# TACJu/Axial-VS

Hardware: AMD Instinct MI355X
Metric: axial-trajectory-attn fwd frames/sec at [B=1,T=4,C=256,H=W=64]; 1/2/4/8 GPU (higher is better)
Workload: dtype f16

## Files before the change

axial_vs_amd/_lib.py:

```python
from __future__ import annotations

import ctypes as C
import os
import threading
from typing import Optional

_HERE = os.path.dirname(os.path.abspath(__file__))
LIB_PATH = os.environ.get("AXVS_LIB_PATH") or os.path.join(_HERE, "libaxvs.so")

AXVS_F16 = 0
AXVS_BF16 = 1
AXVS_F32 = 2
AXVS_U8 = 3
DTYPES = {"f16": AXVS_F16, "fp16": AXVS_F16, "float16": AXVS_F16, "bf16": AXVS_BF16, "bfloat16": AXVS_BF16}

_fp = C.c_void_p


class AxvsTrajParams(C.Structure):
    _fields_ = [(n, _fp) for n in ("q_w", "q_b", "k_w", "k_b", "v_w", "v_b", "proj_q_w", "proj_q_b",
                                   "proj_kv_w", "proj_kv_b", "proj_w", "proj_b")]


class AxvsAxialLayerParams(C.Structure):
# ... 136 lines not shown
class AxvsCnxDownParams(C.Structure):
    _fields_ = [(n, _fp) for n in CNX_DOWN_FIELDS]


class AxvsCnxBlockParams(C.Structure):
    _fields_ = [(n, _fp) for n in CNX_BLOCK_FIELDS]


class AxvsCnxCfg(C.Structure):
    _fields_ = [(n, C.c_int) for n in ("N", "H", "W")] + [(n, C.c_int * 4) for n in ("dims", "depths", "h", "w")] + [("v2", C.c_int)]


class AxvsMsdaParams(C.Structure):
    _fields_ = [(n, _fp) for n in ("value_proj_w", "value_proj_b", "sampling_offsets_w", "sampling_offsets_b",
                                   "attention_weights_w", "attention_weights_b", "output_proj_w", "output_proj_b")]


class AxvsMsdaLayerParams(C.Structure):
    _fields_ = [("self_attn", AxvsMsdaParams)] + [(n, _fp) for n in ("norm1_w", "norm1_b", "linear1_w", "linear1_b", "linear2_w",
                                                                      "linear2_b", "norm2_w", "norm2_b")]


class AxvsConvGnParams(C.Structure):
    _fields_ = [(n, _fp) for n in ("conv_w", "conv_b", "gn_w", "gn_b")]


class AxvsFfnParams(C.Structure):
    _fields_ = [(n, _fp) for n in ("norm1_w", "norm1_b", "linear1_w", "linear1_b", "linear2_w", "linear2_b", "norm2_w", "norm2_b")]


class AxvsFpnLevelParams(C.Structure):
    _fields_ = [(n, _fp) for n in ("lateral_w", "lateral_gn_w", "lateral_gn_b", "output_w", "output_gn_w", "output_gn_b", "mask_w", "mask_b")]


def ptrs(ts) -> C.Array:
    return (C.c_void_p * len(ts))(*[None if t is None else t.data_ptr() for t in ts])


def fill(cls, ptrs):
    ptrs = list(ptrs)
    s, n = _fill(cls, ptrs, 0)
    if n != len(ptrs):
        raise ValueError(f"{cls.__name__} takes {n} pointers, got {len(ptrs)}")
    return s


def _fill(cls, ptrs, i):
    s = cls()
    for name, t in cls._fields_:
        if issubclass(t, C.Structure):
            v, i = _fill(t, ptrs, i)
        elif issubclass(t, C.Array):
            v, i = t(*ptrs[i:i + t._length_]), i + t._length_
        else:
            v, i = (ptrs[i] if i < len(ptrs) else None), i + 1
        setattr(s, name, v)
    return s, i


class AxvsTestGemm(C.Structure):
    _fields_ = [("op", C.c_int), ("a", _fp), ("b", _fp), ("c", _fp), ("M", C.c_longlong), ("N", C.c_int), ("K", C.c_int),
                ("lda", C.c_longlong), ("ldb", C.c_longlong), ("ldc", C.c_longlong), ("al_a", C.c_int), ("al_b", C.c_int), ("al_c", C.c_int),
                ("a2", _fp), ("aff", _fp), ("aff_rows", C.c_int), ("ksteps", C.c_int), ("zsplits", C.c_int), ("bias", _fp), ("mul", C.c_float),
                ("relu", C.c_int), ("drop_seed", C.c_uint), ("drop_site", C.c_uint), ("drop_thr", C.c_uint), ("drop_scale", C.c_float),
                ("beta", C.c_float), ("res", _fp), ("res2", _fp), ("out16", _fp), ("kind16", C.c_int), ("zero_rows", _fp), ("db", _fp),
                ("exact", C.c_int), ("stat_part", _fp), ("stat_shift", _fp), ("stat_nblk", C.c_int), ("stat_blk0", C.c_int),
                ("stat_rows", C.c_int), ("grp_rows", C.c_int), ("grp_ld", C.c_longlong), ("variant", C.c_int)]


TEST_GEMM_OPS = {"nt": 0, "fwd": 1, "wgrad": 2, "dgrad": 3, "tn_direct": 4}


SIGNATURES = {
    "axvs_version": (C.c_int, []),
    "axvs_has_bf16": (C.c_int, []),
    "axvs_last_error": (C.c_char_p, []),
    "axvs_set_status_buffer": (C.c_int, [_fp]),
    "axvs_check_status": (C.c_int, []),
    "axvs_set_sync_buffer": (C.c_int, [_fp, C.c_size_t]),
    "axvs_profile_stages": (C.c_int, [C.POINTER(C.c_void_p), C.c_int]),
    "axvs_profile_stage_count": (C.c_int, []),
    "axvs_profile_stage_name": (C.c_char_p, [C.c_int]),
    "axvs_set_option": (C.c_int, [C.c_char_p, C.c_int]),
    "axvs_traj_packed_bytes": (C.c_size_t, [C.c_int, C.c_int]),
    "axvs_traj_pack": (C.c_int, [C.POINTER(AxvsTrajParams), _fp, C.c_int, C.c_int, C.c_int, _fp]),
    "axvs_axial_layer_packed_bytes": (C.c_size_t, [C.c_int, C.c_int, C.c_int]),
    "axvs_axial_layer_pack": (C.c_int, [C.POINTER(AxvsAxialLayerParams), _fp, C.c_int, C.c_int, C.c_int, C.c_int, _fp]),
    "axvs_traj_attn_workspace_bytes": (C.c_size_t, [C.c_int] * 5),
    "axvs_traj_attn_fwd": (C.c_int, [_fp, _fp, _fp, _fp, _fp, _fp] + [C.c_int] * 6 + [_fp, C.c_size_t, _fp]),
    "axvs_axial_layer_workspace_bytes": (C.c_size_t, [C.c_int] * 7),
    "axvs_axial_layer_fwd": (C.c_int, [_fp, _fp, _fp, _fp] + [C.c_int] * 8 + [_fp, C.c_size_t, _fp, _fp, _fp]),
    "axvs_traj_layer_packed_bytes": (C.c_size_t, [C.c_int] * 3),
    "axvs_traj_layer_pack": (C.c_int, [C.POINTER(AxvsTrajLayerParams), _fp, C.c_int, C.c_int, C.c_int, C.c_int, _fp]),
    "axvs_traj_layer_workspace_bytes": (C.c_size_t, [C.c_int] * 6),
    "axvs_traj_layer_fwd": (C.c_int, [_fp, _fp, _fp, _fp] + [C.c_int] * 7 + [_fp, C.c_size_t, _fp]),
    "axvs_axial_layer_train_saved_bytes": (C.c_size_t, [C.c_int] * 7),
    "axvs_axial_layer_train_scratch_bytes": (C.c_size_t, [C.c_int] * 8),
    "axvs_axial_layer_train_fwd": (C.c_int, [_fp, _fp, _fp, C.POINTER(AxvsAxialLayerParams)] + [C.c_int] * 7 +
                                   [C.c_float, C.c_float, C.c_uint, _fp, C.c_size_t, _fp, C.c_size_t, _fp]),
    "axvs_axial_layer_train_bwd": (C.c_int, [_fp, _fp, _fp, C.POINTER(AxvsAxialLayerParams), C.POINTER(AxvsAxialLayerParams), _fp, _fp] +
                                   [C.c_int] * 7 + [C.c_float, C.c_float, C.c_uint, C.c_int, _fp, C.c_size_t, _fp, C.c_size_t, _fp]),
    "axvs_traj_layer_train_saved_bytes": (C.c_size_t, [C.c_int] * 6),
    "axvs_traj_layer_train_scratch_bytes": (C.c_size_t, [C.c_int] * 7),
    "axvs_traj_layer_train_fwd": (C.c_int, [_fp, _fp, _fp, C.POINTER(AxvsTrajLayerParams)] + [C.c_int] * 6 +
                                  [C.c_float, C.c_float, C.c_uint, _fp, C.c_size_t, _fp, C.c_size_t, _fp]),
    "axvs_traj_layer_train_bwd": (C.c_int, [_fp, _fp, _fp, C.POINTER(AxvsTrajLayerParams), C.POINTER(AxvsTrajLayerParams), _fp, _fp] +
                                  [C.c_int] * 6 + [C.c_float, C.c_float, C.c_uint, C.c_int, _fp, C.c_size_t, _fp, C.c_size_t, _fp]),
    "axvs_cc_module_train_saved_bytes": (C.c_size_t, [C.POINTER(AxvsCCTrainCfg)]),
    "axvs_cc_module_train_scratch_bytes": (C.c_size_t, [C.POINTER(AxvsCCTrainCfg), C.c_int]),
    "axvs_cc_module_train_bn_stats_floats": (C.c_size_t, [C.POINTER(AxvsCCTrainCfg)]),
    "axvs_cc_module_train_fwd": (C.c_int, [_fp] * 5 + [C.POINTER(AxvsCCLayerParams), C.POINTER(AxvsCCHeadParams), C.POINTER(AxvsCCTrainCfg),
                                           _fp, C.c_size_t, _fp, C.c_size_t, _fp]),
    "axvs_cc_module_train_bwd": (C.c_int, [_fp] * 4 + [C.POINTER(AxvsCCLayerParams), C.POINTER(AxvsCCHeadParams), C.POINTER(AxvsCCLayerParams),
                                           C.POINTER(AxvsCCHeadGrads), _fp, C.POINTER(AxvsCCTrainCfg), _fp, C.c_size_t, _fp, C.c_size_t, _fp]),
    "axvs_cc_layers_train_fwd": (C.c_int, [_fp, _fp, C.POINTER(AxvsCCLayerParams), C.POINTER(AxvsCCTrainCfg), _fp, C.c_size_t, _fp, C.c_size_t, _fp]),
    "axvs_cc_layers_train_bwd": (C.c_int, [_fp, _fp, C.POINTER(AxvsCCLayerParams), C.POINTER(AxvsCCLayerParams), _fp, C.POINTER(AxvsCCTrainCfg),
                                           _fp, C.c_size_t, _fp, C.c_size_t, _fp]),
    "axvs_axial_pass_fwd": (C.c_int, [_fp, _fp, _fp, _fp] + [C.c_int] * 9 + [_fp, C.c_size_t, _fp]),
    "axvs_axial_layer_workspace_bytes_ex": (C.c_size_t, [C.c_int] * 9),
    "axvs_axial_layer_sine3d_workspace_bytes": (C.c_size_t, [C.c_int] * 7),
    "axvs_axial_layer_fwd_sine3d": (C.c_int, [_fp, C.POINTER(AxvsSinePos3D), _fp, _fp] + [C.c_int] * 8 + [_fp, C.c_size_t, _fp, _fp, _fp]),
    "axvs_axial_layer_strided_ok": (C.c_int, [C.c_int] * 3),
    "axvs_axial_layer_workspace_bytes_strided": (C.c_size_t, [C.c_int] * 7 + [C.c_longlong]),
    "axvs_axial_layer_fwd_sine3d_strided": (C.c_int, [_fp, C.POINTER(AxvsSinePos3D), _fp, _fp] + [C.c_int] * 8 + [C.c_longlong, _fp, C.c_size_t, _fp]),
    "axvs_ffn_workspace_bytes": (C.c_size_t, [C.c_longlong, C.c_int, C.c_int]),
    "axvs_ffn_fwd": (C.c_int, [_fp, _fp, _fp, C.c_longlong, C.c_int, C.c_int, C.c_int, C.c_int, _fp, C.c_size_t, _fp]),
    "axvs_cc_layer_packed_bytes": (C.c_size_t, []),
    "axvs_cc_layer_pack": (C.c_int, [C.POINTER(AxvsCCLayerParams), _fp, C.c_int, _fp]),
    "axvs_cc_layer_workspace_bytes": (C.c_size_t, [C.c_int] * 3),
    "axvs_cc_layer_fwd": (C.c_int, [_fp, _fp, _fp, C.c_int, C.c_int, C.c_int, C.POINTER(C.c_int), C.c_int, _fp, C.c_size_t, _fp]),
    "axvs_cc_heads_packed_bytes": (C.c_size_t, [C.c_int]),
    "axvs_cc_heads_pack": (C.c_int, [C.POINTER(AxvsCCHeadParams), _fp, C.c_int, C.c_int, _fp]),
    "axvs_cc_heads_workspace_bytes": (C.c_size_t, [C.c_int] * 3),
    "axvs_cc_heads_fwd": (C.c_int, [_fp, _fp, _fp, _fp, _fp] + [C.c_int] * 8 + [_fp, C.c_size_t, _fp]),
    "axvs_ffn_packed_bytes": (C.c_size_t, [C.c_int, C.c_int]),
    "axvs_ffn_pack": (C.c_int, [C.POINTER(AxvsFfnParams), _fp, C.c_int, C.c_int, C.c_int, _fp]),
    "axvs_ffn_packed_fwd": (C.c_int, [_fp, _fp, _fp, C.c_longlong, C.c_int, C.c_int, C.c_int, _fp, C.c_size_t, _fp]),
    "axvs_fpn_level_packed_bytes": (C.c_size_t, [C.c_int] * 3),
    "axvs_fpn_level_pack": (C.c_int, [C.POINTER(AxvsFpnLevelParams), _fp, C.c_int, C.c_int, C.c_int, C.c_int, _fp]),
    "axvs_fpn_level_workspace_bytes": (C.c_size_t, [C.c_int] * 6),
    "axvs_fpn_level_fwd": (C.c_int, [_fp, _fp, C.c_longlong, C.c_longlong, C.c_int, C.c_int, _fp, _fp, _fp] + [C.c_int] * 7 +
                           [C.c_float, C.c_int, _fp, C.c_size_t, _fp]),
    "axvs_conv1x1_gn_packed_bytes": (C.c_size_t, [C.c_int, C.c_int]),
    "axvs_conv1x1_gn_pack": (C.c_int, [C.POINTER(AxvsConvGnParams), _fp, C.c_int, C.c_int, C.c_int, _fp]),
    "axvs_conv1x1_gn_workspace_bytes": (C.c_size_t, [C.c_int] * 4),
    "axvs_conv1x1_gn_fwd": (C.c_int, [_fp, C.c_int, C.c_longlong, C.c_longlong, _fp, C.c_int, C.c_longlong, C.c_longlong, _fp] +
                            [C.c_int] * 5 + [C.c_float, C.c_int, _fp, C.c_size_t, _fp]),
    "axvs_conv1x1_gn_train_saved_bytes": (C.c_size_t, [C.c_int] * 6 + [C.c_longlong, C.c_longlong]),
    "axvs_conv1x1_gn_train_scratch_bytes": (C.c_size_t, [C.c_int] * 6),
    "axvs_conv1x1_gn_train_fwd": (C.c_int, [_fp, C.c_int, C.c_longlong, C.c_longlong, _fp, C.c_int, C.c_longlong, C.c_longlong, C.POINTER(AxvsConvGnParams)] +
                                  [C.c_int] * 5 + [C.c_float, _fp, C.c_size_t, _fp, C.c_size_t, _fp]),
    "axvs_conv1x1_gn_train_bwd": (C.c_int, [_fp, C.c_int, C.c_longlong, C.c_longlong, _fp, C.c_int, C.c_longlong, C.c_longlong, C.POINTER(AxvsConvGnParams),
                                            C.POINTER(AxvsConvGnParams), _fp] + [C.c_int] * 5 + [_fp, C.c_size_t, _fp, C.c_size_t, _fp]),
    "axvs_linear_sum_assignment": (C.c_int, [_fp, _fp, C.c_int, C.c_int, _fp]),
    "axvs_match_embds_workspace_bytes": (C.c_size_t, [C.c_int, C.c_int]),
    "axvs_match_embds": (C.c_int, [_fp, _fp, _fp, C.c_int, C.c_int, _fp, C.c_size_t, _fp]),
    "axvs_match_clips_workspace_bytes": (C.c_size_t, [C.c_int] * 4),
    "axvs_match_clips": (C.c_int, [_fp, _fp] + [C.c_int] * 4 + [_fp, C.c_size_t, _fp]),
    "axvs_linear_sum_assignment_rect": (C.c_int, [_fp, C.c_longlong, C.c_int, C.c_int, C.POINTER(C.c_int), _fp, _fp, C.c_int, _fp]),
    "axvs_video_matcher_workspace_bytes": (C.c_size_t, [C.c_int] * 4 + [C.c_longlong]),
    "axvs_video_matcher": (C.c_int, [C.POINTER(_fp), C.c_int, C.POINTER(_fp), _fp, C.c_int, _fp, C.POINTER(C.c_int)] + [C.c_int] * 4 +
                           [C.c_longlong, C.c_int, C.c_int] + [_fp] * 5 + [_fp, C.c_size_t, _fp]),
    "axvs_set_criterion_saved_bytes": (C.c_size_t, [C.c_int] * 3),
    "axvs_set_criterion_workspace_bytes": (C.c_size_t, [C.c_int] * 4 + [C.c_longlong]),
    "axvs_set_criterion_fwd": (C.c_int, [C.POINTER(_fp), C.POINTER(_fp), _fp, C.c_int, _fp, C.POINTER(C.c_int)] + [_fp] * 4 + [C.c_int] * 5 +
                               [C.c_longlong, C.c_int, C.c_int, _fp, _fp, _fp, C.c_longlong, _fp]),
# ... 181 lines not shown
```

axial_vs_amd/csrc/axvs_api.hip:

```cpp
#include <hip/hip_runtime.h>

#include <algorithm>
#include <cmath>
#include <cstdio>
#include <cstring>
#include <type_traits>

#include "axvs_infer.h"
#include "axvs_attn.h"
#include "axvs_fused.h"
#include "axvs_ffn_split.h"
#include "axvs_ffn_wide.h"
#include "axvs_misc.h"

namespace axvs {
namespace {

constexpr int kMergeSmall = 128;
thread_local int g_generic_only = 0;
thread_local int* g_status = nullptr;
thread_local volatile int* g_status_host = nullptr;
thread_local unsigned g_sync_spin_limit = axvs::kSyncSpinLimit;
thread_local long long g_row_span = 0;
thread_local int g_ffn_wide = 0;
thread_local int g_no_small_tiles = 0;
thread_local int g_ffn_split_pairs = 1;
thread_local int g_spatial_only = 0;
thread_local int g_no_ffn_fusion = 0;
thread_local int g_no_reassoc = 0;
thread_local int g_ffn_gelu = 0;
thread_local unsigned* g_sync = nullptr;
thread_local size_t g_sync_words = 0;
thread_local int g_merge_qkv_any = 0;
thread_local int g_merge_small = kMergeSmall;
thread_local int g_out_dtype = 0;
thread_local int g_no_merge_qkv = 0;
thread_local int g_no_attn_fusion = 0;

constexpr int kSmallBelow = 65;
constexpr int kMergeMid = 1;
constexpr int kQkvSplitUpto = 64;
int cu_count() {
  static thread_local int dev_seen = -1, cus = 0;
  int dev = 0;
  if (hipGetDevice(&dev) != hipSuccess) return 0;
  if (dev != dev_seen) {
    hipDeviceProp_t pr;
    if (hipGetDeviceProperties(&pr, dev) != hipSuccess) return 0;
    cus = pr.multiProcessorCount;
    dev_seen = dev;
  }
  return cus;
}

int status_gate() {
  if (g_status_host != nullptr && (*g_status_host & AXVS_STATUS_SYNC_TIMEOUT))
    return fail(AXVS_ERR_STATE, "an earlier merged q/k/v + trajectory launch gave up waiting for its sibling row tiles (status bit 2, "
                                "AXVS_STATUS_SYNC_TIMEOUT): its outputs are invalid and its sync words are not zero.  Synchronise, zero the sync words "
                                "(axvs_set_sync_buffer contract), clear the status word, then call again -- or run two launches per pass "
                                "(axvs_set_sync_buffer(NULL, 0) / option no_merge_qkv)");
  return AXVS_OK;
}

template <bool BF>
void pack_w(const float* W, u16* out, PackDim nd, PackDim kd, hipStream_t st, int n_off = 0, int n_total = 0) {
  long long total = (long long)nd.padded * kd.padded;
  hipLaunchKernelGGL((pack_weight_kernel<BF>), dim3((unsigned)((total + 255) / 256)), dim3(256), 0, st, W, out, nd, kd, n_off,
                     n_total ? n_total : nd.padded);
}
template <bool BF>
void pack_w3(const float* W, u16* out, PackDim nd, PackDim kd, hipStream_t st, int n_off = 0, int n_total = 0) {
  long long total = (long long)nd.padded * kd.padded;
  hipLaunchKernelGGL((pack_weight_split3_kernel<BF>), dim3((unsigned)((total + 255) / 256)), dim3(256), 0, st, W, out, nd, kd, n_off,
                     n_total ? n_total : nd.padded);
}

template <bool BF>
void pack_ffn(const float* n1w, const float* n1b, const float* l1w, const float* l1b, const float* l2w, const float* l2b,
              const float* n2w, const float* n2b, const LayerPacked& l, int C, int F, hipStream_t st) {
  PackDim plainC{C, C, 0, 0, 0}, plainF{F, F, 0, 0, 0};
  pack_w<BF>(l1w, l.w1, plainF, plainC, st);
  pack_w<BF>(l2w, l.w2, plainC, plainF, st);
  pack_b(l1b, l.b1, plainF, st);
  pack_b(l2b, l.b2, plainC, st);
  pack_b(n1w, l.g1, plainC, st);
  pack_b(n1b, l.be1, plainC, st);
  pack_b(n2w, l.g2, plainC, st);
  pack_b(n2b, l.be2, plainC, st);
}

template <bool BF>
void pack_traj(const AxvsTrajParams& p, const TrajPacked& t, int C, int heads, hipStream_t st) {
  const int d = C / heads, Cp = heads * 32;
  PackDim plainC{C, C, 0, 0, 0}, headC{C, Cp, heads, d, 0}, head2C{2 * C, 2 * Cp, heads, d, 0}, headCp{C, Cp, heads, d, 1};
  pack_w<BF>(p.q_w, t.wq, headC, plainC, st);
  pack_w<BF>(p.k_w, t.wk, headC, plainC, st);
  pack_w<BF>(p.v_w, t.wv, headC, plainC, st);
  pack_w<BF>(p.proj_q_w, t.wpq, headC, headCp, st);
  pack_w<BF>(p.proj_kv_w, t.wpkv, head2C, headCp, st);
  if (d == 32) {
    const dim3 pg((unsigned)(((long long)heads * C * 32 + 255) / 256));
    hipLaunchKernelGGL((pack_wk2t_kernel<BF>), pg, dim3(256), 0, st, p.proj_kv_w, t.wk2t, C, heads);
    hipLaunchKernelGGL((pack_wk2n_kernel<BF>), pg, dim3(256), 0, st, p.proj_kv_w, t.wk2n, C, heads);
    hipLaunchKernelGGL((pack_wv2h_kernel<BF>), pg, dim3(256), 0, st, p.proj_kv_w, t.wv2h, C, heads);
  }
  pack_w<BF>(p.proj_w, t.wp, plainC, headC, st);
  pack_b(p.q_b, t.bq, headC, st);
  pack_b(p.k_b, t.bk, headC, st);
  pack_b(p.v_b, t.bv, headC, st);
  pack_b(p.proj_q_b, t.bpq, headC, st);
  pack_b(p.proj_kv_b, t.bpkv, head2C, st);
  pack_b(p.proj_b, t.bp, plainC, st);
}

struct TrajAttnWs {
  TrajWs tw;
  float* zeros;
};
TrajAttnWs carve_traj_attn_ws(Carver& c, int S, int T, int L, int C, int heads) {
  const long long M = (long long)S * T * L;
  TrajAttnWs w{};
  w.tw = carve_traj_ws(c, M, T, heads, false, padded_rows(M, L));
  w.zeros = c.take<float>((size_t)M * C);
  return w;
}
struct TrajLayerWs {
  TrajWs tw;
  FfnWs f;
};
TrajLayerWs carve_traj_layer_ws(Carver& c, int B, int T, int HW, int C, int heads, int F) {
  const long long M = (long long)B * T * HW;
  TrajLayerWs w{};
  w.tw = carve_traj_ws(c, M, T, heads, false, padded_rows(M, HW));
  w.f = carve_ffn_ws(c, M, C, F);
  return w;
}

}
TrajPlan plan_traj(int S, int T, int L, int C, int heads, bool want_attn, bool same_src, int F, bool may_merge) {
  TrajPlan p{};
  p.may_merge = may_merge;
  const bool kernels = !g_generic_only && C == 256 && heads == 8;
  const bool few_rows_forms = !g_no_small_tiles;
  p.tier = !(kernels && (T <= 8 || (T <= 12 && few_rows_forms))) ? TrajPlan::kGeneric
           : same_src && !g_no_attn_fusion && !want_attn && L >= 8 && L <= 128 ? TrajPlan::kFused : TrajPlan::kTemporalFused;
  p.L = p.tier == TrajPlan::kFused ? pad16(L) : L;
  p.nks = (p.L + 31) / 32;
  p.reassoc = p.tier == TrajPlan::kGeneric && kernels && !g_no_reassoc && T >= 12;
  const int N = T * p.L;
  const long long Mreal = (long long)S * T * L, Mp = (long long)S * N;
  p.qkv = !(kernels && same_src) ? TrajPlan::kQkvGemms : ((Mp + 63) / 64 <= kQkvSplitUpto && few_rows_forms) ? TrajPlan::kQkvKernel3 : TrajPlan::kQkvKernel;
  if (p.tier == TrajPlan::kGeneric) return p;
  p.with_ffn = p.tier == TrajPlan::kFused && F > 0 && !g_no_ffn_fusion && !g_ffn_gelu && T <= 4 && F % 256 == 0 && F <= 4096 &&
               (Mreal >= (long long)kSmallBelow * 64 || !few_rows_forms);
  const long long tiles64 = p.tier == TrajPlan::kFused ? (long long)S * ((N + 63) / 64) : (Mp + 63) / 64;
  p.rows = !p.with_ffn && (tiles64 < kSmallBelow || T > 8) && few_rows_forms ? 16 : T <= 4 ? 64 : 32;
  const bool own_frame = p.rows == 64 && p.L == 64 && T >= 2;
  const auto fits = [&] {
    return p.rows == 64   ? own_frame || tiles64 <= 640 || g_merge_qkv_any
           : p.rows == 32 ? kMergeMid && (kMergeMid == 2 || (long long)S * ((N + 31) / 32) <= cu_count())
                          : g_merge_small && (g_merge_small == 1 || (long long)S * ((N + 15) / 16) <= g_merge_small);
  };
  const bool merge = p.tier == TrajPlan::kFused && may_merge && !g_no_merge_qkv && g_sync != nullptr && (size_t)S <= g_sync_words &&
                     (T <= 4 || p.rows == 32) && p.nks <= (p.rows == 16 ? 4 : 3) && 2 * (long long)heads * 32 * Mp * 2 < (1ll << 32) && fits();
  p.mq = !merge ? 0 : own_frame ? 2 : 1;
  return p;
}
namespace {

bool ffn_wide_pays(long long M) {
  const long long r64 = ((M + kRows - 1) / kRows + 255) / 256, r128 = ((M + kWideRows - 1) / kWideRows + 255) / 256;
  return r64 > 1 && r128 * 11 < r64 * 6;
}

struct FfnPlan {
  enum Kind { kSplit2, kSplit1, kWide, kFused, kGeneric } kind;
  int split;
  bool gelu;
  int oflags;
  const char* refuse;
};
FfnPlan plan_ffn(int C, int heads, int F, long long M, bool has_part, bool strided) {
  FfnPlan p{};
  p.gelu = g_ffn_gelu != 0;
  p.oflags = g_out_dtype ? (g_out_dtype == 1 ? kOutF16 : kOutBf16) : 0;
  const bool kernels = !g_generic_only && C == 256 && heads == 8 && F % 256 == 0 && F <= 4096;
  if (kernels && !g_no_small_tiles && F >= 512)
    p.split = M < (long long)kSmallBelow * 64 ? 1 : (g_ffn_split_pairs && F % 512 == 0 && M <= 88 * 64) ? 2 : 0;
  static_assert(kFfnTiles + (4096 + 5 * 256) * sizeof(float) <= 160 * 1024, "ffn_lds_bytes: every d_ffn the fused FFN kernels take fits the LDS");
  if (!kernels) {
    p.kind = FfnPlan::kGeneric;
    p.refuse = p.oflags ? "layer_out_dtype: a 16-bit output map needs the fused FFN tier (C = 256, 8 heads, d_ffn a multiple of 256 up to 4096)"
               : strided ? "internal: strided frames need the fused FFN kernels" : nullptr;
  } else if (!p.oflags && has_part && p.split) {
    p.kind = p.split == 2 ? FfnPlan::kSplit2 : FfnPlan::kSplit1;
  } else if (!p.oflags && F <= 2048 && (g_ffn_wide == 1 || (g_ffn_wide == 0 && ffn_wide_pays(M)))) {
    p.kind = FfnPlan::kWide;
  } else {
    p.kind = FfnPlan::kFused;
  }
  return p;
}

struct LayerPlan {
  TrajPlan h, w;
  FfnPlan ffn;
  bool pos_in_kernel;
  bool lean_traj() const { return h.tier == TrajPlan::kFused && w.tier == TrajPlan::kFused; }
  bool need_buf2() const { return !w.with_ffn; }
  bool need_ffn_tmp() const { return need_buf2() && ffn.kind == FfnPlan::kGeneric; }
  bool need_ffn_part() const { return need_buf2() && ffn.split != 0; }
};
LayerPlan plan_layer(int B, int T, int H, int W, int C, int heads, int F, bool want_h_attn, bool want_w_attn, bool strided = false) {
  LayerPlan p{};
  p.h = plan_traj(B * W, T, H, C, heads, want_h_attn, true, 0, true);
  p.w = plan_traj(B * H, T, W, C, heads, want_w_attn, true, F, true);
  p.ffn = plan_ffn(C, heads, F, (long long)B * T * H * W, true, strided);
  p.pos_in_kernel = p.h.qkv != TrajPlan::kQkvGemms && p.w.qkv != TrajPlan::kQkvGemms;
  return p;
}

struct AxialWs {
  TrajWs tw;
  float *buf1, *buf2;
  u16 *y16, *h16;
  float* ffn_part;
  float* pos;
};
AxialWs carve_axial_ws(Carver& c, const LayerPlan& plan, bool sine, long long span, int B, int T, int H, int W, int C, int heads, int F) {
  const long long M = (long long)B * T * H * W;
  AxialWs w{};
  w.tw = carve_traj_ws(c, M, T, heads, plan.lean_traj(), std::max(padded_rows(M, H), padded_rows(M, W)));
  w.buf1 = c.take<float>((size_t)span * C);
  if (plan.need_buf2()) w.buf2 = c.take<float>((size_t)span * C);
  if (plan.need_ffn_tmp()) {
    w.y16 = c.take<u16>((size_t)M * C);
    w.h16 = c.take<u16>((size_t)M * F);
  }
  if (plan.need_ffn_part()) w.ffn_part = c.take<float>((size_t)(F / 256) * M * C);
  if (sine && !plan.pos_in_kernel) w.pos = c.take<float>((size_t)M * C);
  return w;
}

template <bool BF, int NKS>
int launch_attn(const TrajWs& w, float* attn, int S, int N, int T, int L, int heads, long long Mp, hipStream_t st) {
  const size_t per_frame = (size_t)NKS * 32 * 32 * 2 * sizeof(u16);
  const int tch = (int)((150 * 1024) / per_frame) < T ? (int)((150 * 1024) / per_frame) : T;
  const size_t lds = per_frame * tch;
  if (int rc = ensure_max_lds(reinterpret_cast<const void*>(&spatial_attn_kernel<BF, NKS>))) return rc;
  const int nwaves = (N + 31) / 32 >= 8 ? 8 : (N + 31) / 32;
  dim3 grid((N + 32 * nwaves - 1) / (32 * nwaves), heads, S);
  hipLaunchKernelGGL((spatial_attn_kernel<BF, NKS>), grid, dim3(64 * nwaves), lds, st, w.q16, w.k16, w.v16, w.x16, attn, N, T, L,
                     heads, Mp, tch);
  return AXVS_OK;
}

template <int N, class F>
int by_int(int i, F&& f) {
  if constexpr (N == 0) return fail(AXVS_ERR_ARG, "internal: no kernel is instantiated for %d", i);
  else return i == N ? f(std::integral_constant<int, N>{}) : by_int<N - 1>(i, f);
}

template <bool BF>
int launch_temporal(const TrajPlan& pl, int nks, const TrajWs& w, const TrajPacked& p, const float* res, float* out, RowMap rm, long long Mp, int N,
                    int T, float scale, hipStream_t st, const FfnArgs* fa = nullptr, const OwnQkv* oq = nullptr) {
  const int wt = ((g_row_span ? g_row_span : Mp) * 256 * 4 < (1ll << 32) ? 1 : 0) | (g_spatial_only && nks > 0 ? (oq ? g_spatial_only : 1) << 1 : 0) |
                 (fa != nullptr && g_out_dtype ? (g_out_dtype == 1 ? kOutF16 : kOutBf16) : 0);
  if (oq && !(nks > 0 && T <= 8)) return fail(AXVS_ERR_ARG, "internal: own q,k,v need the in-kernel spatial half and T <= 8");
  return by_int<12>(T, [&](auto t) {
    constexpr int kT = decltype(t)::value;
    if (pl.rows == 16) return launch_temporal_n<BF, kT, 1>(nks, w, p, res, out, rm, Mp, N, pl.L, scale, st, fa, wt, oq);
    if constexpr (kT <= 4) return launch_temporal_n<BF, kT, 4>(nks, w, p, res, out, rm, Mp, N, pl.L, scale, st, fa, wt, oq);
    else if constexpr (kT <= 8) return launch_temporal_n<BF, kT, 2>(nks, w, p, res, out, rm, Mp, N, pl.L, scale, st, fa, wt, oq);
    else return fail(AXVS_ERR_ARG, "fused temporal kernel supports T <= 8");
  });
}

template <bool BF>
int run_traj(const TrajPlan& pl, const float* qsrc, const float* ksrc, const float* vsrc, const float* qk_add, const float* res, float* out,
             float* attn, const TrajPacked& p, const TrajWs& w, RowMap rm, int S, int T, int L, int C, int heads,
             hipStream_t st, int pass = 0, const FfnArgs* ffn = nullptr, float* ffn_out = nullptr, const PosGen* posgen = nullptr) {
  static const char* const kNames[3][9] = {
      {"qkv_proj", "spatial_attn", "proj_q", "proj_kv", "temporal_attn", "proj", "temporal_fused", "traj_fused", "qkv+traj"},
      {"h.qkv_proj", "h.spatial_attn", "h.proj_q", "h.proj_kv", "h.temporal_attn", "h.proj", "h.temporal_fused", "h.traj_fused", "h.qkv+traj"},
      {"w.qkv_proj", "w.spatial_attn", "w.proj_q", "w.proj_kv", "w.temporal_attn", "w.proj", "w.temporal_fused", "w.traj_fused", "w.qkv+traj"}};
  const char* const* nm = kNames[pass];
  if (pl.may_merge)
    if (int rc = status_gate()) return rc;
  const int Cp = heads * 32, d = C / heads;
  if ((long long)S * T * L * T > 2147483647LL / 4) return fail(AXVS_ERR_ARG, "too many tokens for 32-bit row indices");
  const float scale = 1.0f / sqrtf((float)d);
  const float qscale = scale * 1.4426950408889634f;
  if (pl.L != L) {
    rm.Lv = L;
    rm.L = pl.L;
    rm.N = T * pl.L;
  }
  const int N = T * pl.L;
  const long long Mp = (long long)S * N;
  const int M = (int)Mp;
  const FfnArgs* const fa = pl.with_ffn ? ffn : nullptr;
  float* const dst = pl.with_ffn ? ffn_out : out;
  const PosGen pg = posgen ? *posgen : PosGen{};
  if (pl.mq) {
    const OwnQkv oq{qsrc, qk_add, pg, p.wq, p.wk, p.wv, p.bq, p.bk, p.bv, qscale, g_sync, g_status, g_sync_spin_limit};
    if (int rc = launch_temporal<BF>(pl, pl.nks, w, p, res, dst, rm, Mp, N, T, scale, st, fa, &oq)) return rc;
    mark(st, pl.with_ffn ? "w.qkv+traj+ffn" : nm[8]);
    return AXVS_OK;
  }
  if (pl.qkv == TrajPlan::kQkvGemms) {
    if (posgen) return fail(AXVS_ERR_ARG, "internal: generated positions need the fused QKV kernel");
    ALoadRowsF32<BF> aq{qsrc, qk_add, rm, M, C}, ak{ksrc, qk_add, rm, M, C}, av{vsrc, nullptr, rm, M, C};
    launch_gemm<BF>(aq, p.wq, EpiBlocked16<BF>{w.q16, Mp, p.bq, qscale, Cp, 0}, M, Cp, C, st);
    launch_gemm<BF>(ak, p.wk, EpiBlocked16<BF>{w.k16, Mp, p.bk, 1.f, 0, 0}, M, Cp, C, st);
    launch_gemm<BF>(av, p.wv, EpiBlocked16<BF>{w.v16, Mp, p.bv, 1.f, 0, 0}, M, Cp, C, st);
  } else {
    if (int rc = ensure_max_lds(reinterpret_cast<const void*>(&qkv_fused_kernel<BF>))) return rc;
    hipLaunchKernelGGL((qkv_fused_kernel<BF>), dim3((unsigned)((Mp + 63) / 64), pl.qkv == TrajPlan::kQkvKernel3 ? 3 : 1), dim3(512), kQkvLdsBytes, st, qsrc, qk_add, rm,
                       p.wq, p.wk, p.wv, p.bq, p.bk, p.bv, w.q16, w.k16, w.v16, Mp, qscale,
                       pl.tier == TrajPlan::kFused ? w.vt16 : (u16*)nullptr, N, pl.L, T, pl.nks, pg,
                       2 * (long long)Cp * Mp * 2 < (1ll << 32) ? 1 : 0 , g_status);
  }
  mark(st, nm[0]);
  if (pl.tier == TrajPlan::kFused) {
    if (int rc = launch_temporal<BF>(pl, pl.nks, w, p, res, dst, rm, Mp, N, T, scale, st, fa)) return rc;
    mark(st, pl.with_ffn ? "w.traj_fused+ffn" : nm[7]);
    return AXVS_OK;
  }

  if (pl.nks <= 8) {
    if (int rc = by_int<8>(pl.nks, [&](auto nks) { return launch_attn<BF, decltype(nks)::value>(w, attn, S, N, T, L, heads, Mp, st); })) return rc;
  } else {
    if (attn != nullptr) return fail(AXVS_ERR_ARG, "attention maps are not available for frames of more than 256 keys (L=%d)", L);
    if (int rc = ensure_max_lds(reinterpret_cast<const void*>(&spatial_attn_long_kernel<BF>))) return rc;
    const int nwaves = (N + 31) / 32 >= 8 ? 8 : (N + 31) / 32;
    dim3 grid((N + 32 * nwaves - 1) / (32 * nwaves), heads, S);
    hipLaunchKernelGGL((spatial_attn_long_kernel<BF>), grid, dim3(64 * nwaves), (size_t)2 * 256 * 32 * sizeof(u16), st, w.q16, w.k16, w.v16,
                       w.x16, N, T, L, heads, Mp);
  }
  mark(st, nm[1]);

  if (pl.tier == TrajPlan::kTemporalFused) {
    if (int rc = launch_temporal<BF>(pl, 0, w, p, res, out, rm, Mp, N, T, scale, st)) return rc;
    mark(st, nm[6]);
    return AXVS_OK;
  }
  ALoadBlocked<BF> adiag{w.x16, Mp * T, M, T, N, L};
  launch_gemm<BF>(adiag, p.wpq, EpiRowsF32{w.q2, nullptr, p.bpq, identity_map(Mp), Cp, scale}, M, Cp, Cp, st);
  mark(st, nm[2]);
  if (pl.reassoc) {
    float* U = w.kv2;
    float* Z = w.kv2 + (size_t)Mp * heads * Cp;
    {
      GemmBatch<ALoadRowsLd<BF>, EpiRowsF32, 8> gb;
      for (int h = 0; h < 8; ++h) {
        gb.al[h] = ALoadRowsLd<BF>{w.q2, Cp, h * 32, M};
        gb.W[h] = p.wk2n + (size_t)h * Cp * 32;
        gb.epi[h] = EpiRowsF32{U + h * Cp, nullptr, nullptr, identity_map(Mp), heads * Cp, 1.f};
      }
      launch_gemm_batched<BF>(gb, M, Cp, 32, st);
    }
    hipLaunchKernelGGL((temporal_stream_kernel<BF>), dim3((unsigned)((Mp + 3) / 4)), dim3(256), 0, st, (const float*)U, (const u16*)w.x16, Z,
                       (long long)M, Mp, T);
    mark(st, nm[3]);
    {
      GemmBatch<ALoadRowsLd<BF>, EpiBlocked16<BF>, 8> gb;
      for (int h = 0; h < 8; ++h) {
        gb.al[h] = ALoadRowsLd<BF>{Z, heads * Cp, h * Cp, M};
        gb.W[h] = p.wv2h + (size_t)h * Cp * 32;
        gb.epi[h] = EpiBlocked16<BF>{w.o16, Mp, p.bpkv + Cp + h * 32, 1.f, 0, 0};
        gb.epi[h].n_off = h * 32;
      }
      launch_gemm_batched<BF>(gb, M, 32, Cp, st);
    }
    mark(st, nm[4]);
  } else {
    ALoadBlocked<BF> aall{w.x16, Mp * T, M * T, 0, 1, 1};
    launch_gemm<BF>(aall, p.wpkv, EpiRowsF32{w.kv2, nullptr, p.bpkv, identity_map(Mp * T), 2 * Cp, 1.f}, M * T, 2 * Cp, Cp, st);
    mark(st, nm[3]);
    const long long threads = Mp * heads * 8;
    hipLaunchKernelGGL((temporal_attn_kernel<BF>), dim3((unsigned)((threads + 255) / 256)), dim3(256), 0, st, w.q2, w.kv2,
                       w.o16, Mp, T, heads);
    mark(st, nm[4]);
  }
  ALoadBlocked<BF> ao{w.o16, Mp, M, 0, 1, 1};
  launch_gemm<BF>(ao, p.wp, EpiRowsF32{out, res, p.bp, rm, C, 1.f}, M, C, Cp, st);
  mark(st, nm[5]);
  return AXVS_OK;
}

template <class F>
auto by_gelu(bool gelu, F&& f) {
  return gelu ? f(std::true_type{}) : f(std::false_type{});
}

template <bool BF>
int run_ffn(const FfnPlan& pl, float* X, float* out, const LayerPacked& p, long long M, int C, int F, float* tmp, u16* y16, u16* h16,
            hipStream_t st, float* part = nullptr ,
            RowStride rs = RowStride{0, 0} ) {
  if (pl.refuse) return fail(AXVS_ERR_ARG, "%s", pl.refuse);
  const unsigned tiles = (unsigned)((M + kRows - 1) / kRows);
  switch (pl.kind) {
    case FfnPlan::kSplit2:
    case FfnPlan::kSplit1: {
      const int rc = by_gelu(pl.gelu, [&](auto g) {
        const auto launch = [&](auto cpw) {
          const auto kern = &ffn_split_kernel<BF, decltype(g)::value, decltype(cpw)::value>;
          if (int rc = ensure_max_lds(reinterpret_cast<const void*>(kern))) return rc;
          hipLaunchKernelGGL(kern, dim3(tiles, F / (256 * decltype(cpw)::value)), dim3(512), kFfnSplitLds, st, (const float*)X, p.w1, p.b1, p.w2, p.g1, p.be1, part, M, F, rs);
          return (int)AXVS_OK;
        };
        return pl.kind == FfnPlan::kSplit2 ? launch(std::integral_constant<int, 2>{}) : launch(std::integral_constant<int, 1>{});
      });
      if (rc != AXVS_OK) return rc;
      hipLaunchKernelGGL(ffn_finish_kernel, dim3((unsigned)((M + 3) / 4)), dim3(256), 0, st, (const float*)X, (const float*)part, p.b2, p.g1, p.be1,
                         p.g2, p.be2, out, M, F / 256, rs);
      break;
    }
    case FfnPlan::kWide: {
      const int rc = by_gelu(pl.gelu, [&](auto g) {
        const auto kern = &ffn_wide_kernel<BF, decltype(g)::value>;
        if (int rc = ensure_max_lds(reinterpret_cast<const void*>(kern))) return rc;
        hipLaunchKernelGGL(kern, dim3((unsigned)((M + kWideRows - 1) / kWideRows)), dim3(512), ffn_wide_lds_bytes(F), st, (const float*)X, p.w1, p.b1, p.w2, p.b2,
                           p.g1, p.be1, p.g2, p.be2, out, M, F, rs);
        return (int)AXVS_OK;
      });
      if (rc != AXVS_OK) return rc;
      break;
    }
    case FfnPlan::kFused: {
      const int rc = by_gelu(pl.gelu, [&](auto g) {
        const auto kern = &ffn_fused_kernel<BF, decltype(g)::value>;
        if (int rc = ensure_max_lds(reinterpret_cast<const void*>(kern))) return rc;
        hipLaunchKernelGGL(kern, dim3(tiles), dim3(512), ffn_lds_bytes(F), st, X, p.w1, p.b1, p.w2, p.b2, p.g1, p.be1, p.g2, p.be2, out, M, F, rs, pl.oflags);
        return (int)AXVS_OK;
      });
      if (rc != AXVS_OK) return rc;
      break;
    }
    case FfnPlan::kGeneric: {
      const unsigned lnblocks = (unsigned)((M + 3) / 4);
      hipLaunchKernelGGL((layernorm_kernel<BF>), dim3(lnblocks), dim3(256), 0, st, X, p.g1, p.be1, tmp, y16, M, C, 1e-5f);
      mark(st, "norm1");
      ALoadBlocked<BF> ay{y16, M, (int)M, 0, 1, 1};
      launch_gemm<BF>(ay, p.w1, EpiBlocked16<BF>{h16, M, p.b1, 1.f, 0, pl.gelu ? 2 : 1}, (int)M, F, C, st);
      mark(st, "ffn.linear1");
      ALoadBlocked<BF> ah{h16, M, (int)M, 0, 1, 1};
      launch_gemm<BF>(ah, p.w2, EpiRowsF32{X, tmp, p.b2, identity_map(M), C, 1.f}, (int)M, C, F, st);
      mark(st, "ffn.linear2");
      hipLaunchKernelGGL((layernorm_kernel<BF>), dim3(lnblocks), dim3(256), 0, st, X, p.g2, p.be2, out, (u16*)nullptr, M, C, 1e-5f);
      mark(st, "norm2");
      return AXVS_OK;
    }
  }
  mark(st, "norm1+ffn+norm2");
  return AXVS_OK;
}

template <bool BF>
int traj_attn_fwd_t(const float* query, const float* key, const float* value, float* out, float* attn, const void* packed,
                    int S, int T, int L, int C, int heads, void* ws, hipStream_t st) {
  Carver pc(const_cast<void*>(packed));
  TrajPacked p = carve_traj(pc, C, heads);
  Carver wc(ws);
  const TrajAttnWs w = carve_traj_attn_ws(wc, S, T, L, C, heads);
  if (hipMemsetAsync(w.zeros, 0, (size_t)S * T * L * C * sizeof(float), st) != hipSuccess) return fail(AXVS_ERR_LAUNCH, "memset failed");
  RowMap rm{T * L, L, 1, (long long)T * L, L, 1, 0};
  const TrajPlan plan = plan_traj(S, T, L, C, heads, attn != nullptr, query == key && value == query, 0, false);
  int rc = run_traj<BF>(plan, query, key, value, nullptr, w.zeros, out, attn, p, w.tw, rm, S, T, L, C, heads, st);
  return rc != AXVS_OK ? rc : last_launch_status();
}

PosGen make_posgen(const AxvsSinePos3D& sp, int T, int H, int W, int C, int l_is_h) {
  PosGen pg{};
  pg.mode = 1;
  pg.l_is_h = l_is_h;
  const float eps = 1e-6f;
  pg.zs = sp.normalize ? sp.scale / ((float)T + eps) : 1.f;
  pg.ys = sp.normalize ? sp.scale / ((float)H + eps) : 1.f;
  pg.xs = sp.normalize ? sp.scale / ((float)W + eps) : 1.f;
  pg.n = C / 2;
  pg.ke_yx = -log2f(sp.temperature) * 2.f / (float)pg.n;
  pg.ke_z = -log2f(sp.temperature) * 2.f / (float)C;
  pg.level = sp.level_embed;
  return pg;
}

template <bool BF>
int axial_layer_fwd_t(const float* src, const float* pos, float* out, const void* packed, int B, int T, int H, int W, int C,
                      int heads, int F, void* ws, float* h_attn, float* w_attn, hipStream_t st, const AxvsSinePos3D* sine = nullptr,
                      int which = 0 ,
                      long long fs = 0 ) {
  Carver pc(const_cast<void*>(packed));
  LayerPacked p = carve_layer(pc, C, heads, F);
  const long long M = (long long)B * T * H * W;
  const long long span = fs ? ((long long)B * T - 1) * fs + (long long)H * W : M;
  struct SpanGuard { SpanGuard(long long v) { g_row_span = v; } ~SpanGuard() { g_row_span = 0; } } span_guard(fs ? span : 0);
  if (g_out_dtype && (fs != 0 || which == 1))
    return fail(AXVS_ERR_ARG, "layer_out_dtype: a 16-bit output map exists for the whole layer / its width pass on contiguous frames only");
  Carver wc(ws);
  const LayerPlan plan = plan_layer(B, T, H, W, C, heads, F, h_attn != nullptr, w_attn != nullptr, fs != 0);
  const AxialWs w = carve_axial_ws(wc, plan, sine != nullptr, span, B, T, H, W, C, heads, F);
  float* buf1 = w.buf1;
  float* const scratch1 = buf1;
  const long long sB = fs ? (long long)T * fs : (long long)T * H * W, sT = fs ? fs : (long long)H * W;

  g_prof_next = 0;
  mark(st, "begin");
  PosGen pgh{}, pgw{};
  const PosGen *ph = nullptr, *pw = nullptr;
  if (sine) {
    if (plan.pos_in_kernel) {
      pgh = make_posgen(*sine, T, H, W, C, 1);
      pgw = make_posgen(*sine, T, H, W, C, 0);
      ph = &pgh;
      pw = &pgw;
    } else {
      float* pbuf = w.pos;
// ... 25 lines not shown
  int rc2 = run_ffn<BF>(plan.ffn, w.buf2, out, p, M, C, F, scratch1, w.y16, w.h16, st, w.ffn_part, fs ? RowStride{H * W, fs - (long long)H * W} : RowStride{0, 0});
  if (rc2 != AXVS_OK) return rc2;
  return last_launch_status();
}

template <bool BF>
int traj_layer_fwd_t(const float* src, const float* pos, float* out, const void* packed, int B, int T, int HW, int C, int heads, int F,
                     void* ws, hipStream_t st) {
  Carver pc(const_cast<void*>(packed));
  TrajPacked pt = carve_traj(pc, C, heads);
  LayerPacked pf = carve_ffn(pc, C, F);
  const long long M = (long long)B * T * HW;
  Carver wc(ws);
  const TrajLayerWs w = carve_traj_layer_ws(wc, B, T, HW, C, heads, F);
  g_prof_next = 0;
  mark(st, "begin");
  RowMap rm{T * HW, HW, 1, (long long)T * HW, HW, 1, 0};
  int rc = run_traj<BF>(plan_traj(B, T, HW, C, heads, false, true, 0, false), src, src, src, pos, src, w.f.x, nullptr, pt, w.tw, rm, B, T, HW, C, heads, st, 0);
  if (rc != AXVS_OK) return rc;
  rc = run_ffn<BF>(plan_ffn(C, heads, F, M, false, false), w.f.x, out, pf, M, C, F, w.f.tmp, w.f.y16, w.f.h16, st);
  return rc != AXVS_OK ? rc : last_launch_status();
}

}

void pack_w(int dtype, const float* W, u16* out, PackDim nd, PackDim kd, hipStream_t st, int n_off, int n_total) {
  by_dtype(dtype, [&](auto bf) { pack_w<bf()>(W, out, nd, kd, st, n_off, n_total); });
}
void pack_w3(int dtype, const float* W, u16* out, PackDim nd, PackDim kd, hipStream_t st, int n_off, int n_total) {
  by_dtype(dtype, [&](auto bf) { pack_w3<bf()>(W, out, nd, kd, st, n_off, n_total); });
}
void pack_b(const float* b, float* out, PackDim nd, hipStream_t st) {
  hipLaunchKernelGGL(pack_bias_kernel, dim3((nd.padded + 255) / 256), dim3(256), 0, st, b, out, nd);
}
void copy_f32(const float* src, float* dst, int n, hipStream_t st) {
  PackDim d{n, n, 0, 0, 0};
  pack_b(src, dst, d, st);
}
void pack_traj(int dtype, const AxvsTrajParams& p, const TrajPacked& t, int C, int heads, hipStream_t st) {
  by_dtype(dtype, [&](auto bf) { pack_traj<bf()>(p, t, C, heads, st); });
}
void pack_ffn(int dtype, const float* n1w, const float* n1b, const float* l1w, const float* l1b, const float* l2w, const float* l2b,
              const float* n2w, const float* n2b, const LayerPacked& l, int C, int F, hipStream_t st) {
  by_dtype(dtype, [&](auto bf) { pack_ffn<bf()>(n1w, n1b, l1w, l1b, l2w, l2b, n2w, n2b, l, C, F, st); });
}
int run_traj(int dtype, const TrajPlan& pl, const float* qsrc, const float* ksrc, const float* vsrc, const float* qk_add, const float* res,
             float* out, float* attn, const TrajPacked& p, const TrajWs& w, RowMap rm, int S, int T, int L, int C, int heads, hipStream_t st) {
  return by_dtype(dtype, [&](auto bf) { return run_traj<bf()>(pl, qsrc, ksrc, vsrc, qk_add, res, out, attn, p, w, rm, S, T, L, C, heads, st); });
}
int ffn_rows(int dtype, const FfnWs& w, float* out, const LayerPacked& p, long long M, int C, int heads, int d_ffn, hipStream_t st) {
  int rc = by_dtype(dtype, [&](auto bf) { return run_ffn<bf()>(plan_ffn(C, heads, d_ffn, M, false, false), w.x, out, p, M, C, d_ffn, w.tmp, w.y16, w.h16, st); });
  return rc != AXVS_OK ? rc : last_launch_status();
}
int ffn_rows(int dtype, const float* x, float* out, const LayerPacked& p, long long M, int C, int heads, int d_ffn, void* workspace, hipStream_t st) {
  Carver wc(workspace);
  const FfnWs w = carve_ffn_ws(wc, M, C, d_ffn);
  if (hipMemcpyAsync(w.x, x, (size_t)M * C * sizeof(float), hipMemcpyDeviceToDevice, st) != hipSuccess)
    return fail(AXVS_ERR_LAUNCH, "copy failed");
  g_prof_next = 0;
  return ffn_rows(dtype, w, out, p, M, C, heads, d_ffn, st);
}
void layernorm_rows(int dtype, const float* X, const float* gamma, const float* beta, float* Y, u16* Y16, long long M, int C, hipStream_t st) {
  by_dtype(dtype, [&](auto bf) { hipLaunchKernelGGL((layernorm_kernel<bf()>), dim3((unsigned)((M + 3) / 4)), dim3(256), 0, st, X, gamma, beta, Y, Y16, M, C, 1e-5f); });
}
template void launch_gemm<false, ALoadBlocked<false>, EpiBlocked16<false>>(const ALoadBlocked<false>&, const u16*, const EpiBlocked16<false>&, int, int, int, hipStream_t, int);
#ifdef AXVS_WITH_BF16
template void launch_gemm<true, ALoadBlocked<true>, EpiBlocked16<true>>(const ALoadBlocked<true>&, const u16*, const EpiBlocked16<true>&, int, int, int, hipStream_t, int);
#endif

}

using namespace axvs;

extern "C" {

int axvs_version(void) { return 1; }
int axvs_has_bf16(void) { return kBF ? 1 : 0; }

int axvs_profile_stages(void** events, int capacity) {
  g_prof_events = reinterpret_cast<hipEvent_t*>(events);
  g_prof_cap = events ? capacity : 0;
  return kMaxStages;
}
int axvs_profile_stage_count(void) { return g_prof_next < kMaxStages ? g_prof_next : kMaxStages; }
const char* axvs_profile_stage_name(int i) { return (i >= 0 && i < kMaxStages && g_stage_names[i]) ? g_stage_names[i] : ""; }

#if defined(AXVS_STAMPS) && defined(AXVS_STAMPS_QKV)
int axvs_debug_read_stamps(unsigned long long* host, int n) {
  return (int)hipMemcpyFromSymbol(host, HIP_SYMBOL(axvs::g_stamps), sizeof(unsigned long long) * n);
}
#endif

int axvs_set_option(const char* key, int value) {
  if (!key) return fail(AXVS_ERR_ARG, "null option key");
  if (!strcmp(key, "generic_only")) { g_generic_only = value; return AXVS_OK; }
  if (!strcmp(key, "no_attn_fusion")) { g_no_attn_fusion = value; return AXVS_OK; }
  if (!strcmp(key, "no_ffn_fusion")) { g_no_ffn_fusion = value; return AXVS_OK; }
  if (!strcmp(key, "ffn_gelu")) { g_ffn_gelu = value; return AXVS_OK; }
  if (!strcmp(key, "train_valu")) { g_train_valu = value; return AXVS_OK; }
  if (!strcmp(key, "train_exact")) { g_train_exact = value; return AXVS_OK; }
  if (!strcmp(key, "train_amp")) {
    if (value < 0 || value > 2) return fail(AXVS_ERR_ARG, "train_amp: 0 (off), 1 (bf16 products) or 2 (fp16 products)");
    g_train_amp = value;
    return AXVS_OK;
  }
  if (!strcmp(key, "spatial_only")) { g_spatial_only = value; return AXVS_OK; }
  if (!strcmp(key, "cc_aspp_affine")) { g_cc_aspp_affine = value ? 1 : 0; return AXVS_OK; }
  if (!strcmp(key, "cc_last_heads_only")) { g_cc_last_only = value; return AXVS_OK; }
  if (!strcmp(key, "no_merge_qkv")) { g_no_merge_qkv = value; return AXVS_OK; }
  if (!strcmp(key, "merge_qkv_any")) { g_merge_qkv_any = value; return AXVS_OK; }
  if (!strcmp(key, "layer_out_dtype")) {
    if (value < 0 || value > 2) return fail(AXVS_ERR_ARG, "layer_out_dtype: 0 (fp32), 1 (f16) or 2 (bf16)");
    g_out_dtype = value;
    return AXVS_OK;
  }
  if (!strcmp(key, "sync_spin_limit")) { g_sync_spin_limit = value > 0 ? (unsigned)value : axvs::kSyncSpinLimit; return AXVS_OK; }
  if (!strcmp(key, "plan_force")) {
    g_no_small_tiles = (value & 1) ? 1 : 0;
    g_ffn_wide = (value & 2) ? 1 : (value & 4) ? 2 : 0;
    g_ffn_split_pairs = (value & 8) ? 0 : 1;
    g_merge_small = (value & 16) ? 0 : (value & 32) ? 1 : kMergeSmall;
    g_no_reassoc = (value & 64) ? 1 : 0;
    return AXVS_OK;
  }
  return fail(AXVS_ERR_ARG, "unknown option");
}
const char* axvs_last_error(void) { return g_err; }

int axvs_set_status_buffer(int* device_word) {
  g_status = device_word;
  g_status_host = nullptr;
  if (device_word != nullptr) {
    hipPointerAttribute_t at{};
    if (hipPointerGetAttributes(&at, device_word) == hipSuccess && at.type == hipMemoryTypeHost && at.hostPointer != nullptr)
      g_status_host = static_cast<volatile int*>(at.hostPointer);
    else
      (void)hipGetLastError();
  }
  return AXVS_OK;
}

int axvs_check_status(void) { return status_gate(); }

int axvs_set_sync_buffer(unsigned* device_words, size_t n_words) {
  if (device_words != nullptr && n_words == 0) return fail(AXVS_ERR_ARG, "empty sync buffer");
  g_sync = device_words;
  g_sync_words = device_words ? n_words : 0;
  return AXVS_OK;
}

size_t axvs_traj_packed_bytes(int C, int heads) { return carved([&](Carver& c) { carve_traj(c, C, heads); }); }

int axvs_traj_pack(const AxvsTrajParams* p, void* packed, int C, int heads, int dtype, void* stream) {
  if (int rcd = check_dtype(dtype)) return rcd;
  if (!p || !packed) return fail(AXVS_ERR_ARG, "null pointer");
  if (int rc = check_cfg(C, heads)) return rc;
  Carver c(packed);
  TrajPacked t = carve_traj(c, C, heads);
  hipStream_t st = static_cast<hipStream_t>(stream);
  pack_traj(dtype, *p, t, C, heads, st);
  return last_launch_status();
}

size_t axvs_axial_layer_packed_bytes(int C, int heads, int d_ffn) { return carved([&](Carver& c) { carve_layer(c, C, heads, d_ffn); }); }

int axvs_axial_layer_pack(const AxvsAxialLayerParams* p, void* packed, int C, int heads, int d_ffn, int dtype, void* stream) {
  if (int rcd = check_dtype(dtype)) return rcd;
  if (!p || !packed) return fail(AXVS_ERR_ARG, "null pointer");
  if (int rc = check_cfg(C, heads)) return rc;
  if (int rc = check_ffn(d_ffn)) return rc;
  Carver c(packed);
  LayerPacked l = carve_layer(c, C, heads, d_ffn);
  hipStream_t st = static_cast<hipStream_t>(stream);
  pack_traj(dtype, p->height_attn, l.th, C, heads, st);
  pack_traj(dtype, p->width_attn, l.tw, C, heads, st);
  pack_ffn(dtype, *p, l, C, d_ffn, st);
  return last_launch_status();
}

size_t axvs_traj_attn_workspace_bytes(int S, int T, int L, int C, int heads) { return carved([&](Carver& c) { carve_traj_attn_ws(c, S, T, L, C, heads); }); }

int axvs_traj_attn_fwd(const float* query, const float* key, const float* value, float* out, float* space_attn,
                       const void* packed, int S, int T, int L, int C, int heads, int dtype, void* workspace,
                       size_t workspace_bytes, void* stream) {
  if (int rcd = check_dtype(dtype)) return rcd;
  if (!query || !key || !value || !out || !packed || !workspace) return fail(AXVS_ERR_ARG, "null pointer");
  if (S <= 0 || T <= 0 || L <= 0) return fail(AXVS_ERR_ARG, "empty shape S=%d T=%d L=%d", S, T, L);
  if (int rc = check_cfg(C, heads)) return rc;
  if (int rc = check_ws(workspace_bytes, axvs_traj_attn_workspace_bytes(S, T, L, C, heads))) return rc;
  hipStream_t st = static_cast<hipStream_t>(stream);
  return by_dtype(dtype, [&](auto bf) { return traj_attn_fwd_t<bf()>(query, key, value, out, space_attn, packed, S, T, L, C, heads, workspace, st); });
}

static size_t layer_ws_bytes(int B, int T, int H, int W, int C, int heads, int d_ffn, int want_attn_maps, int sine_pos, long long span) {
  return carved([&](Carver& c) { carve_axial_ws(c, plan_layer(B, T, H, W, C, heads, d_ffn, want_attn_maps != 0, want_attn_maps != 0), sine_pos != 0, span, B, T, H, W, C, heads, d_ffn); });
}
size_t axvs_axial_layer_workspace_bytes_ex(int B, int T, int H, int W, int C, int heads, int d_ffn, int want_attn_maps, int sine_pos) {
  return layer_ws_bytes(B, T, H, W, C, heads, d_ffn, want_attn_maps, sine_pos, (long long)B * T * H * W);
}

size_t axvs_axial_layer_workspace_bytes_strided(int B, int T, int H, int W, int C, int heads, int d_ffn, long long frame_stride_rows) {
  return layer_ws_bytes(B, T, H, W, C, heads, d_ffn, 0, 1, ((long long)B * T - 1) * frame_stride_rows + (long long)H * W);
}

int axvs_axial_layer_strided_ok(int C, int heads, int d_ffn) {
// ... 146 lines not shown
```

axial_vs_amd/csrc/axvs_common.h:

```cpp
#pragma once
#include <hip/hip_runtime.h>
#include <stdint.h>

namespace axvs {

typedef unsigned short u16;
typedef unsigned short u16x4 __attribute__((ext_vector_type(4)));
typedef unsigned short u16x8 __attribute__((ext_vector_type(8)));
typedef short s16x4 __attribute__((ext_vector_type(4)));
typedef _Float16 f16x8 __attribute__((ext_vector_type(8)));
typedef __bf16 bf16x8 __attribute__((ext_vector_type(8)));
typedef float f32x4 __attribute__((ext_vector_type(4)));

constexpr int kWave = 64;
constexpr int kBlk = 32;
constexpr int kLsapMax = 512;

template <bool BF>
struct H16;

template <>
struct H16<false> {
  static __device__ __forceinline__ u16 from_f32(float x) { return __builtin_bit_cast(u16, (_Float16)x); }
  static __device__ __forceinline__ float to_f32(u16 x) { return (float)__builtin_bit_cast(_Float16, x); }
// ... 77 lines not shown
  if (rm.Lv) l = min(l, rm.Lv - 1);
  return b * rm.sB + t * rm.sT + l * rm.sL + o * rm.sO;
}
__device__ __forceinline__ bool row_exists(const RowMap& rm, int mp) {
  if (!rm.Lv) return true;
  const int n = mp % rm.N;
  return n % rm.L < rm.Lv;
}

struct RowStride {
  int hw;
  long long extra;
  __device__ __forceinline__ long long row(long long m) const { return hw ? m + (m / hw) * extra : m; }
};

__device__ __forceinline__ float gelu_exact(float x) { return 0.5f * x * (1.f + erff(x * 0.70710678118654752f)); }

inline int row_align(const void* base, long long ld, long long step) {
  const unsigned long long a = reinterpret_cast<unsigned long long>(base);
  if (a % 16 == 0 && ld % 4 == 0 && step % 4 == 0) return 4;
  if (a % 8 == 0 && ld % 2 == 0 && step % 2 == 0) return 2;
  return 1;
}

typedef float f32x4_u __attribute__((ext_vector_type(4), aligned(4)));
__device__ __forceinline__ float4 ldg4(const float* p, int valid, int ) {
  if (valid >= 4) {
    const f32x4_u v = *reinterpret_cast<const f32x4_u*>(p);
    return float4{v.x, v.y, v.z, v.w};
  }
  float4 r = {0.f, 0.f, 0.f, 0.f};
  if (valid > 0) r.x = p[0];
  if (valid > 1) r.y = p[1];
  if (valid > 2) r.z = p[2];
  return r;
}
__device__ __forceinline__ void stg4(float* p, float4 v, int valid, int ) {
  if (valid >= 4) {
    *reinterpret_cast<f32x4_u*>(p) = f32x4_u{v.x, v.y, v.z, v.w};
    return;
  }
  if (valid > 0) p[0] = v.x;
  if (valid > 1) p[1] = v.y;
  if (valid > 2) p[2] = v.z;
}

__device__ __forceinline__ long long nat_row_coords(const RowMap& rm, int mp, int l_is_h, int* packed) {
  int s = mp / rm.N, n = mp - s * rm.N;
  int b = s / rm.Loff, o = s - b * rm.Loff;
  int t = n / rm.L, l = n - t * rm.L;
  if (rm.Lv) l = min(l, rm.Lv - 1);
  *packed = t | ((l_is_h ? l : o) << 8) | ((l_is_h ? o : l) << 20);
  return b * rm.sB + t * rm.sT + l * rm.sL + o * rm.sO;
}

struct PosGen {
  int mode;
  int l_is_h;
  float zs, ys, xs;
  float ke_yx, ke_z;
  int n;
  const float* level;
};

struct PosGenLane {
  float f0, f1, g0, g1;
  float lv[4];
  int xside;
  __device__ __forceinline__ void init(const PosGen& pg, int c0) {
    const float inv2pi = 0.15915494309189535f;
    xside = c0 >= pg.n;
    const int cc = c0 - (xside ? pg.n : 0);
    f0 = __builtin_amdgcn_exp2f(pg.ke_yx * (float)(cc >> 1)) * inv2pi;
    f1 = __builtin_amdgcn_exp2f(pg.ke_yx * (float)((cc >> 1) + 1)) * inv2pi;
    g0 = __builtin_amdgcn_exp2f(pg.ke_z * (float)(c0 >> 1)) * inv2pi;
    g1 = __builtin_amdgcn_exp2f(pg.ke_z * (float)((c0 >> 1) + 1)) * inv2pi;
    if (pg.level) {
      const float4 l = *reinterpret_cast<const float4*>(pg.level + c0);
      lv[0] = l.x; lv[1] = l.y; lv[2] = l.z; lv[3] = l.w;
    } else {
      lv[0] = lv[1] = lv[2] = lv[3] = 0.f;
    }
  }
  __device__ __forceinline__ float4 eval(const PosGen& pg, int packed) const {
    const float z = (float)((packed & 255) + 1) * pg.zs;
    const float u = xside ? (float)(((packed >> 20) & 4095) + 1) * pg.xs : (float)(((packed >> 8) & 4095) + 1) * pg.ys;
    const float a0 = __builtin_amdgcn_fractf(u * f0), a1 = __builtin_amdgcn_fractf(u * f1);
    const float b0 = __builtin_amdgcn_fractf(z * g0), b1 = __builtin_amdgcn_fractf(z * g1);
    return float4{__builtin_amdgcn_sinf(a0) + __builtin_amdgcn_sinf(b0) + lv[0], __builtin_amdgcn_cosf(a0) + __builtin_amdgcn_cosf(b0) + lv[1],
                  __builtin_amdgcn_sinf(a1) + __builtin_amdgcn_sinf(b1) + lv[2], __builtin_amdgcn_cosf(a1) + __builtin_amdgcn_cosf(b1) + lv[3]};
  }
};

__device__ __forceinline__ long long blk_off(long long R, long long r, int k) {
  return ((long long)(k >> 5) * R + r) * kBlk + (k & 31);
}

__device__ __forceinline__ long long wblk_off(long long R, long long r, int k) {
  const long long Rp = (R + 15) & ~15ll;
#ifdef AXVS_WEIGHT_ROWS
  return ((long long)(k >> 5) * Rp + r) * kBlk + (k & 31);
#endif
  return ((long long)(k >> 5) * Rp + (r & ~15ll)) * kBlk + ((k >> 3) & 3) * 128 + (r & 15) * 8 + (k & 7);
}

__device__ __forceinline__ int swz_chunk(int row, int g) {
  return g ^ ((4 - ((row >> 2) & 3)) & 3);
}

template <int CTRL>
__device__ __forceinline__ float dpp_mov(float v) {
  return __uint_as_float(__builtin_amdgcn_update_dpp(0u, __float_as_uint(v), CTRL, 0xF, 0xF, true));
}
__device__ __forceinline__ float lane_xor1(float v) { return dpp_mov<0xB1>(v); }
__device__ __forceinline__ float lane_xor2(float v) { return dpp_mov<0x4E>(v); }
__device__ __forceinline__ float lane_hmirror(float v) { return dpp_mov<0x141>(v); }
__device__ __forceinline__ float lane_mirror(float v) { return dpp_mov<0x140>(v); }
__device__ __forceinline__ float lane_xor16(float v) {
  auto r = __builtin_amdgcn_permlane16_swap(__float_as_uint(v), __float_as_uint(v), false, false);
  return __uint_as_float((threadIdx.x & 16) ? r[0] : r[1]);
}
__device__ __forceinline__ float lane_xor32(float v) {
  auto r = __builtin_amdgcn_permlane32_swap(__float_as_uint(v), __float_as_uint(v), false, false);
  return __uint_as_float((threadIdx.x & 32) ? r[0] : r[1]);
}
__device__ __forceinline__ float row16_sum(float v) {
  v += lane_xor1(v);
  v += lane_xor2(v);
  v += lane_hmirror(v);
  v += lane_mirror(v);
  return v;
}
__device__ __forceinline__ float max3(float a, float b, float c) {
  float r;
  asm("v_max3_f32 %0, %1, %2, %3" : "=v"(r) : "v"(a), "v"(b), "v"(c));
  return r;
}
__device__ __forceinline__ float groups_sum(float v) {
  auto r = __builtin_amdgcn_permlane16_swap(__float_as_uint(v), __float_as_uint(v), false, false);
  v = __uint_as_float(r[0]) + __uint_as_float(r[1]);
  r = __builtin_amdgcn_permlane32_swap(__float_as_uint(v), __float_as_uint(v), false, false);
  return __uint_as_float(r[0]) + __uint_as_float(r[1]);
}
__device__ __forceinline__ float groups_max(float v) {
  auto r = __builtin_amdgcn_permlane16_swap(__float_as_uint(v), __float_as_uint(v), false, false);
  v = fmaxf(__uint_as_float(r[0]), __uint_as_float(r[1]));
  r = __builtin_amdgcn_permlane32_swap(__float_as_uint(v), __float_as_uint(v), false, false);
  return fmaxf(__uint_as_float(r[0]), __uint_as_float(r[1]));
}
__device__ __forceinline__ float fmaximum(float a, float b) { return __builtin_elementwise_maximum(a, b); }
__device__ __forceinline__ float groups_maximum(float v) {
  auto r = __builtin_amdgcn_permlane16_swap(__float_as_uint(v), __float_as_uint(v), false, false);
  v = fmaximum(__uint_as_float(r[0]), __uint_as_float(r[1]));
  r = __builtin_amdgcn_permlane32_swap(__float_as_uint(v), __float_as_uint(v), false, false);
  return fmaximum(__uint_as_float(r[0]), __uint_as_float(r[1]));
}
__device__ __forceinline__ float wave_sum(float v) { return groups_sum(row16_sum(v)); }

__device__ __forceinline__ float wave_xor_max(float v, int m) { return fmaxf(v, __shfl_xor(v, m, kWave)); }
__device__ __forceinline__ float wave_xor_sum(float v, int m) { return v + __shfl_xor(v, m, kWave); }

typedef unsigned int u32x4 __attribute__((ext_vector_type(4)));
typedef unsigned int u32x2 __attribute__((ext_vector_type(2)));
struct WtBuf {
  __amdgpu_buffer_rsrc_t rsrc;
  __device__ __forceinline__ explicit WtBuf(const void* base)
      : rsrc(__builtin_amdgcn_make_buffer_rsrc(const_cast<void*>(base), 0, -1, 0x00020000)) {}
  __device__ __forceinline__ void store16(unsigned byte_off, u16x8 v) const {
    __builtin_amdgcn_raw_buffer_store_b128(__builtin_bit_cast(u32x4, v), rsrc, byte_off, 0, 16);
  }
  __device__ __forceinline__ void store16(unsigned byte_off, float4 v) const {
    __builtin_amdgcn_raw_buffer_store_b128(__builtin_bit_cast(u32x4, v), rsrc, byte_off, 0, 16);
  }
  __device__ __forceinline__ void store8(unsigned byte_off, u16x4 v) const {
// ... 84 lines not shown
```

axial_vs_amd/csrc/axvs_fused.h:

```cpp
#pragma once
#include <type_traits>

#include "axvs_common.h"

namespace axvs {

constexpr int kRows = 64;
constexpr int kTileElems = kRows * 32;

__device__ __forceinline__ int act_off(int kb, int row, int c) { return (kb * kRows + row) * 32 + swz_chunk(row, c) * 8; }

__device__ __forceinline__ u16x8 act_frag(const u16* tile, int kb, int mt, int fi, int fg) {
  return *reinterpret_cast<const u16x8*>(tile + act_off(kb, mt * 16 + fi, fg));
}

__device__ __forceinline__ u16x8 w_frag(const u16* __restrict__ W, int NR, int kb, int nrow, int fg) {
  return *reinterpret_cast<const u16x8*>(W + wblk_off(NR, nrow, kb * 32 + fg * 8));
}

__device__ __forceinline__ u16x8 w_frag_u(const u16* __restrict__ W, int NR, int kb, int nrow16, int lane) {
  const long long blk = ((long long)kb * ((NR + 15) & ~15) + nrow16) * 32;
  return *reinterpret_cast<const u16x8*>(W + blk + lane * 8);
}

// ... 9 lines not shown
#pragma unroll
  for (int j = 0; j < KB; ++j) {
    const int kb = (j + rot) & (KB - 1);
    u16x8 b[MT];
#pragma unroll
    for (int mt = 0; mt < MT; ++mt) b[mt] = act_frag(tile, kb, mt, fi, fg);
#pragma unroll
    for (int nt = 0; nt < NT; ++nt)
#pragma unroll
      for (int mt = 0; mt < MT; ++mt) acc[nt][mt] = H16<BF>::mfma(wf[nt][j], b[mt], acc[nt][mt]);
  }
}

struct NoKStamps {};
struct KStamps8 { unsigned long long t[8]; };
template <bool BF, int NT, int MT, int KB, int NTN, class KS = NoKStamps>
__device__ __forceinline__ void gemm_phase_pf(f32x4 (&acc)[NT][MT], const u16x8 (&wf)[NT][KB], const u16* tile, int fi, int fg,
                                              int rot, u16x8 (&wnext)[NTN][KB], const u16* __restrict__ Wn, int NRn, int kb0n,
                                              int nrow0n, int rotn, [[maybe_unused]] KS* ks = nullptr ) {
  u16x8 bcur[MT], bnxt[MT];
#pragma unroll
  for (int mt = 0; mt < MT; ++mt) bcur[mt] = act_frag(tile, rot & (KB - 1), mt, fi, fg);
#pragma unroll
  for (int j = 0; j < KB; ++j) {
    if (j + 1 < KB) {
      const int kb = (j + 1 + rot) & (KB - 1);
#pragma unroll
      for (int mt = 0; mt < MT; ++mt) bnxt[mt] = act_frag(tile, kb, mt, fi, fg);
    }
#pragma unroll
    for (int nt = 0; nt < NTN; ++nt) wnext[nt][j] = w_frag(Wn, NRn, kb0n + ((j + rotn) & (KB - 1)), nrow0n + nt * 16 + fi, fg);
#pragma unroll
    for (int nt = 0; nt < NT; ++nt)
#pragma unroll
      for (int mt = 0; mt < MT; ++mt) acc[nt][mt] = H16<BF>::mfma(wf[nt][j], bcur[mt], acc[nt][mt]);
    __builtin_amdgcn_sched_barrier(0);
    if constexpr (!std::is_same<KS, NoKStamps>::value) {
      if (ks) {
        asm volatile("s_memtime %0\n\ts_waitcnt lgkmcnt(0)" : "=s"(ks->t[j])::"memory");
        __builtin_amdgcn_sched_barrier(0);
      }
    }
#pragma unroll
    for (int mt = 0; mt < MT; ++mt) bcur[mt] = bnxt[mt];
  }
}


constexpr int kEpiLd = 256 + 4;

__device__ __forceinline__ void epi_put(float* tile, int row, int n, f32x4 v) {
  *reinterpret_cast<float4*>(tile + row * kEpiLd + n) = float4{v[0], v[1], v[2], v[3]};
}

template <int NT, int KB>
__device__ __forceinline__ void load_wfrags(u16x8 (&wf)[NT][KB], const u16* __restrict__ W, int NR, int kb0, int nrow0, int fi, int fg,
                                            int rot = 0) {
#pragma unroll
  for (int j = 0; j < KB; ++j)
#pragma unroll
    for (int nt = 0; nt < NT; ++nt) wf[nt][j] = w_frag(W, NR, kb0 + ((j + rot) & (KB - 1)), nrow0 + nt * 16 + fi, fg);
}

#if defined(AXVS_STAMPS) && defined(AXVS_STAMPS_FFN)
#define FSTAMP_DECL unsigned long long fst_[16] = {}
#define FSTAMP(s)                                                                          \
  do {                                                                                     \
    __builtin_amdgcn_sched_barrier(0);                                                     \
    asm volatile("s_memtime %0\n\ts_waitcnt lgkmcnt(0)" : "=s"(fst_[s])::"memory");      \
    __builtin_amdgcn_sched_barrier(0);                                                     \
  } while (0)
#define FSTAMP_FLUSH(n)                                                                    \
  do {                                                                                     \
    if (blockIdx.x < 8 && (threadIdx.x & 63) == 0)                                         \
      for (int i_ = 0; i_ < (n); ++i_) ::axvs::g_stamps[i_ * 64 + (blockIdx.x & 7) * 8 + (threadIdx.x >> 6)] = fst_[i_]; \
  } while (0)
#else
#define FSTAMP_DECL
#define FSTAMP(s)
#define FSTAMP_FLUSH(n)
#endif

constexpr int kOutF16 = 16, kOutBf16 = 32, kOut16Mask = kOutF16 | kOutBf16;

struct FfnLds {
  float* xtile;
  u16* ytile;
  u16* htile;
  float* par;
};

struct FfnArgs {
  const u16 *W1, *W2;
  const float *b1, *b2, *g1, *be1, *g2, *be2;
  int F;
};

__device__ __forceinline__ void ffn_stage_params(const FfnLds& l, const float* __restrict__ b1, const float* __restrict__ b2,
                                                 const float* __restrict__ g1, const float* __restrict__ be1,
                                                 const float* __restrict__ g2, const float* __restrict__ be2, int F, int tid) {
  for (int i = tid; i < F; i += 512) {
    l.par[i] = b1[i];
    lds_fence();
  }
  if (tid < 256) {
    float* q = l.par + F;
    q[tid] = b2[tid];
    q[256 + tid] = g1[tid];
    q[512 + tid] = be1[tid];
    q[768 + tid] = g2[tid];
    q[1024 + tid] = be2[tid];
  }
}

struct NoRows { float4 v[8]; };
template <bool BF, class RowOff, bool GELU = false, bool PRE = false>
__device__ __forceinline__ void ffn_body(const FfnLds& l, u16x8 (&w1f)[2][8], const u16* __restrict__ W1, const u16* __restrict__ W2,
                                         float* __restrict__ out, RowOff row_off, int F, int rot, int crot, int tid, int wt = 0,
                                         const NoRows& pre = NoRows{}) {
  constexpr int C = 256, KB = 8;
  const int lane = tid & 63, wave = tid >> 6, fi = lane & 15, fg = lane >> 4;
  const float* sb1 = l.par;
  const float* sb2 = l.par + F;
  const float *sg1 = sb2 + C, *sbe1 = sb2 + 2 * C, *sg2 = sb2 + 3 * C, *sbe2 = sb2 + 4 * C;
  const int nchunk = F / 256;
  u16x8 w2f[2][KB];
  FSTAMP_DECL;
  FSTAMP(0);

  {
    const float4 gg = *reinterpret_cast<const float4*>(sg1 + lane * 4), bb = *reinterpret_cast<const float4*>(sbe1 + lane * 4);
#pragma unroll
    for (int rr = 0; rr < 8; ++rr) {
      const int r = wave * 8 + rr;
      float4 v;
      if constexpr (PRE) v = pre.v[rr];
      else v = *reinterpret_cast<const float4*>(l.xtile + r * kEpiLd + lane * 4);
      const float mu = wave_sum(v.x + v.y + v.z + v.w) * (1.f / C);
      const float a = v.x - mu, b = v.y - mu, c = v.z - mu, d = v.w - mu;
      const float rstd = rsqrtf(wave_sum(a * a + b * b + c * c + d * d) * (1.f / C) + 1e-5f);
      const f32x4 y = {a * rstd * gg.x + bb.x, b * rstd * gg.y + bb.y, c * rstd * gg.z + bb.z, d * rstd * gg.w + bb.w};
      *reinterpret_cast<float4*>(l.xtile + r * kEpiLd + lane * 4) = float4{y[0], y[1], y[2], y[3]};
      act_store4<BF>(l.ytile, lane * 4, r, y);
      if (rr == 3) lds_fence();
    }
  }
  FSTAMP(1);
  __syncthreads();
  FSTAMP(2);

  f32x4 acc2[2][4];
#pragma unroll
  for (int a = 0; a < 2; ++a)
#pragma unroll
    for (int b = 0; b < 4; ++b) acc2[a][b] = f32x4{0.f, 0.f, 0.f, 0.f};

#if defined(AXVS_STAMPS) && defined(AXVS_STAMPS_FFNK)
  KStamps8 kst1{}, kst2{};
#endif
#if defined(AXVS_STAMPS) && defined(AXVS_STAMPS_FFNC)
  KStamps8 ccur{}, cprev{};
#define CSTAMP(i) do { __builtin_amdgcn_sched_barrier(0); asm volatile("s_memtime %0\n\ts_waitcnt lgkmcnt(0)" : "=s"(ccur.t[i])::"memory"); __builtin_amdgcn_sched_barrier(0); } while (0)
#else
#define CSTAMP(i)
#endif
  for (int ci = 0; ci < nchunk; ++ci) {
#if defined(AXVS_STAMPS) && defined(AXVS_STAMPS_FFNC)
    cprev = ccur;
#endif
    CSTAMP(0);
    const int c = (ci + crot) % nchunk;
#if defined(AXVS_STAMPS) && defined(AXVS_STAMPS_FFNK)
    if (ci == AXVS_STAMPS_FFNK) { FSTAMP(14); }
#endif
    const int cn = (min(ci + 1, nchunk - 1) + crot) % nchunk;
    f32x4 acc1[2][4];
#pragma unroll
    for (int a = 0; a < 2; ++a)
#pragma unroll
      for (int b = 0; b < 4; ++b) acc1[a][b] = f32x4{0.f, 0.f, 0.f, 0.f};
#if defined(AXVS_STAMPS) && defined(AXVS_STAMPS_FFNK)
    gemm_phase_pf<BF, 2, 4, KB, 2, KStamps8>(acc1, w1f, l.ytile, fi, fg, rot, w2f, W2, C, c * 8, wave * 32, rot, ci == AXVS_STAMPS_FFNK ? &kst1 : nullptr);
#else
    gemm_phase_pf<BF, 2, 4, KB, 2>(acc1, w1f, l.ytile, fi, fg, rot, w2f, W2, C, c * 8, wave * 32, rot);
#endif
    if (ci == 0) FSTAMP(3);
    CSTAMP(1);
    if (ci > 0) __syncthreads();
    CSTAMP(2);
#pragma unroll
    for (int nt = 0; nt < 2; ++nt) {
      const int hn = c * 256 + wave * 32 + nt * 16 + fg * 4;
      const float4 bias = *reinterpret_cast<const float4*>(sb1 + hn);
#pragma unroll
      for (int mt = 0; mt < 4; ++mt) {
        f32x4 v = acc1[nt][mt];
        if constexpr (GELU) {
          v[0] = gelu_exact(v[0] + bias.x); v[1] = gelu_exact(v[1] + bias.y);
          v[2] = gelu_exact(v[2] + bias.z); v[3] = gelu_exact(v[3] + bias.w);
        } else {
          v[0] = fmaxf(v[0] + bias.x, 0.f); v[1] = fmaxf(v[1] + bias.y, 0.f);
          v[2] = fmaxf(v[2] + bias.z, 0.f); v[3] = fmaxf(v[3] + bias.w, 0.f);
        }
        act_store4<BF>(l.htile, wave * 32 + nt * 16 + fg * 4, mt * 16 + fi, v);
      }
    }
    if (ci == 0) FSTAMP(4);
    CSTAMP(3);
    __syncthreads();
    CSTAMP(4);
    if (ci == 0) FSTAMP(5);
    f32x4 part[2][4];
#pragma unroll
    for (int a = 0; a < 2; ++a)
#pragma unroll
      for (int b = 0; b < 4; ++b) part[a][b] = f32x4{0.f, 0.f, 0.f, 0.f};
#if defined(AXVS_STAMPS) && defined(AXVS_STAMPS_FFNK)
    if (ci == AXVS_STAMPS_FFNK) { FSTAMP(13); }
    gemm_phase_pf<BF, 2, 4, KB, 2, KStamps8>(part, w2f, l.htile, fi, fg, rot, w1f, W1, F, 0, cn * 256 + wave * 32, rot, ci == AXVS_STAMPS_FFNK ? &kst2 : nullptr);
#else
    gemm_phase_pf<BF, 2, 4, KB, 2>(part, w2f, l.htile, fi, fg, rot, w1f, W1, F, 0, cn * 256 + wave * 32, rot);
#endif
#pragma unroll
    for (int a = 0; a < 2; ++a)
#pragma unroll
        for (int b = 0; b < 4; ++b) acc2[a][b] = ci == 0 ? part[a][b] : acc2[a][b] + part[a][b];
    CSTAMP(5);
    if (ci == 0) FSTAMP(6);
    if (ci == 1) FSTAMP(7);
    if (ci == 2) FSTAMP(8);
  }
  FSTAMP(9);

#pragma unroll
  for (int nt = 0; nt < 2; ++nt) {
    const int n = wave * 32 + nt * 16 + fg * 4;
    const float4 b = *reinterpret_cast<const float4*>(sb2 + n);
#pragma unroll
    for (int mt = 0; mt < 4; ++mt) {
      float* p = l.xtile + (mt * 16 + fi) * kEpiLd + n;
      const float4 y = *reinterpret_cast<const float4*>(p);
      *reinterpret_cast<float4*>(p) = float4{y.x + acc2[nt][mt][0] + b.x, y.y + acc2[nt][mt][1] + b.y, y.z + acc2[nt][mt][2] + b.z,
                                             y.w + acc2[nt][mt][3] + b.w};
    }
    lds_fence();
  }
  FSTAMP(10);
  __syncthreads();
  FSTAMP(11);
  {
    const float4 g2v = *reinterpret_cast<const float4*>(sg2 + lane * 4), be2v = *reinterpret_cast<const float4*>(sbe2 + lane * 4);
#pragma unroll
    for (int i = 0; i < 8; ++i) {
      const int r = wave * 8 + i;
      const float4 v = *reinterpret_cast<const float4*>(l.xtile + r * kEpiLd + lane * 4);
      const float mu = wave_sum(v.x + v.y + v.z + v.w) * (1.f / C);
      const float d0 = v.x - mu, d1 = v.y - mu, d2 = v.z - mu, d3 = v.w - mu;
      const float rstd = rsqrtf(wave_sum(d0 * d0 + d1 * d1 + d2 * d2 + d3 * d3) * (1.f / C) + 1e-5f);
      const long long off = row_off(r);
      if (off >= 0) {
        const float4 y = float4{d0 * rstd * g2v.x + be2v.x, d1 * rstd * g2v.y + be2v.y, d2 * rstd * g2v.z + be2v.z, d3 * rstd * g2v.w + be2v.w};
        if (wt & kOut16Mask) {
          const f32x4 yv = {y.x, y.y, y.z, y.w};
          const u16x4 h = (wt & kOutBf16) ? cvt4<true>(yv) : cvt4<false>(yv);
          u16* o16 = reinterpret_cast<u16*>(out);
          if (wt & 1) WtBuf(o16).store8((unsigned)((off + lane * 4) * 2), h);
          else *reinterpret_cast<u16x4*>(o16 + off + lane * 4) = h;
        } else if (wt & 1) WtBuf(out).store16((unsigned)((off + lane * 4) * 4), y);
        else *reinterpret_cast<float4*>(out + off + lane * 4) = y;
      }
      if (i == 3) lds_fence();
    }
  }
  FSTAMP(12);
  FSTAMP_FLUSH(16);
#if defined(AXVS_STAMPS) && defined(AXVS_STAMPS_FFNK)
  if (blockIdx.x < 8 && (threadIdx.x & 63) == 0)
    for (int i_ = 0; i_ < 8; ++i_) {
      ::axvs::g_stamps[(16 + i_) * 64 + (blockIdx.x & 7) * 8 + (threadIdx.x >> 6)] = kst1.t[i_];
      ::axvs::g_stamps[(24 + i_) * 64 + (blockIdx.x & 7) * 8 + (threadIdx.x >> 6)] = kst2.t[i_];
    }
#endif
#if defined(AXVS_STAMPS) && defined(AXVS_STAMPS_FFNC)
  if (blockIdx.x < 8 && (threadIdx.x & 63) == 0)
    for (int i_ = 0; i_ < 8; ++i_) {
      ::axvs::g_stamps[(32 + i_) * 64 + (blockIdx.x & 7) * 8 + (threadIdx.x >> 6)] = cprev.t[i_];
      ::axvs::g_stamps[(40 + i_) * 64 + (blockIdx.x & 7) * 8 + (threadIdx.x >> 6)] = ccur.t[i_];
    }
#endif
}

template <bool BF, bool GELU = false>
__global__ __launch_bounds__(512) void ffn_fused_kernel(const float* __restrict__ X, const u16* __restrict__ W1,
                                                        const float* __restrict__ b1, const u16* __restrict__ W2,
                                                        const float* __restrict__ b2, const float* __restrict__ g1,
                                                        const float* __restrict__ be1, const float* __restrict__ g2,
                                                        const float* __restrict__ be2, float* __restrict__ out,
                                                        long long M, int F, RowStride rs, int oflags = 0 ) {
  constexpr int C = 256, KB = 8;
  extern __shared__ __attribute__((aligned(16))) char smem_c[];
  FfnLds l;
  l.xtile = reinterpret_cast<float*>(smem_c);
  l.ytile = reinterpret_cast<u16*>(smem_c + (size_t)kRows * kEpiLd * sizeof(float));
  l.htile = l.ytile + KB * kTileElems;
  l.par = reinterpret_cast<float*>(l.htile + KB * kTileElems);
  const int tid = threadIdx.x, lane = tid & 63, wave = tid >> 6, fi = lane & 15, fg = lane >> 4;
  const long long m0 = (long long)blockIdx.x * kRows;
  const int nchunk = F / 256;
  constexpr int rot = 0, crot = 0;
  u16x8 w1f[2][KB];
  load_wfrags<2, KB>(w1f, W1, F, 0, crot * 256 + wave * 32, fi, fg, rot);
  ffn_stage_params(l, b1, b2, g1, be1, g2, be2, F, tid);
  {
    float4 rows[8];
#pragma unroll
    for (int rr = 0; rr < 8; ++rr) {
      const long long m = min(m0 + wave * 8 + rr, M - 1);
      rows[rr] = *reinterpret_cast<const float4*>(X + rs.row(m) * C + lane * 4);
    }
#pragma unroll
    for (int rr = 0; rr < 8; ++rr) {
      *reinterpret_cast<float4*>(l.xtile + (wave * 8 + rr) * kEpiLd + lane * 4) = rows[rr];
      if (rr == 3) lds_fence();
    }
  }
  __syncthreads();
  auto row_off = [=](int r) { return m0 + r < M ? rs.row(m0 + r) * C : -1ll; };
  ffn_body<BF, decltype(row_off), GELU>(l, w1f, W1, W2, out, row_off, F, rot, crot, tid, oflags);
}

constexpr size_t kFfnTiles = (size_t)kRows * kEpiLd * sizeof(float) + 2 * 8 * kTileElems * sizeof(u16);
inline size_t ffn_lds_bytes(int F) { return kFfnTiles + (size_t)(F + 5 * 256) * sizeof(float); }



}

namespace axvs {

template <int T, int MT, bool FFN = false>
constexpr size_t temporal_tile_bytes() {
  size_t xt = (size_t)T * 8 * MT * 16 * 32 * sizeof(u16);
  size_t epi = (size_t)8 * MT * 16 * 32 * sizeof(u16) + (size_t)MT * 16 * kEpiLd * sizeof(float);
  if (FFN) epi += (size_t)8 * MT * 16 * 32 * sizeof(u16);
  return xt > epi ? xt : epi;
}
template <int T, int MT, bool FFN = false, int MQ = 0>
constexpr size_t temporal_lds_bytes(int F = 0) {
  return temporal_tile_bytes<T, MT, FFN>() + 3 * 256 * sizeof(float) + (FFN ? (size_t)(F + 5 * 256) * sizeof(float) : 0) +
         (MQ ? 3 * 256 * sizeof(float) : 0);
}

struct OwnQkv {
  const float* src;
  const float* pos;
  PosGen pg;
  const u16 *Wq, *Wk, *Wv;
  const float *bq, *bk, *bv;
  float qscale;
  unsigned* sync;
  int* status;
  unsigned spin_limit;
};
constexpr unsigned kSyncSpinLimit = 1u << 22;

template <int MT>
__device__ __forceinline__ int xt_off(int f, int kb, int row, int c) {
  return ((f * 8 + kb) * (MT * 16) + row) * 32 + swz_chunk(row, c) * 8;
}

template <bool BF, int MT, bool REFILL, bool SWAP = false>
__device__ __forceinline__ void sweep8(f32x4 (&acc)[2][MT], u16x8 (&wf)[2][8], const u16* xt, const int (&bbase)[MT], int kbstride,
                                       const u16* __restrict__ Wn, int NRn, int nrow0n, int fi, int fg) {
  constexpr int LA = MT <= 2 ? 2 : 1;
  u16x8 b[LA + 1][MT];
#pragma unroll
  for (int l = 0; l < LA; ++l)
#pragma unroll
    for (int mt = 0; mt < MT; ++mt) b[l][mt] = *reinterpret_cast<const u16x8*>(xt + bbase[mt] + l * kbstride);
#pragma unroll
  for (int j = 0; j < 8; ++j) {
    if (j + LA < 8) {
#pragma unroll
      for (int mt = 0; mt < MT; ++mt) b[(j + LA) % (LA + 1)][mt] = *reinterpret_cast<const u16x8*>(xt + bbase[mt] + (j + LA) * kbstride);
    }
#pragma unroll
    for (int nt = 0; nt < 2; ++nt)
#pragma unroll
      for (int mt = 0; mt < MT; ++mt)
        acc[nt][mt] = SWAP ? H16<BF>::mfma(b[j % (LA + 1)][mt], wf[nt][j], acc[nt][mt])
                           : H16<BF>::mfma(wf[nt][j], b[j % (LA + 1)][mt], acc[nt][mt]);
    if (REFILL) {
#pragma unroll
      for (int nt = 0; nt < 2; ++nt) wf[nt][j] = w_frag(Wn, NRn, j, nrow0n + nt * 16 + fi, fg);
    }
    __builtin_amdgcn_sched_barrier(0);
  }
}

template <bool BF, int T, int MT, int NKS = 0, bool FFN = false, int MQ = 0>
__global__ __launch_bounds__(512) void temporal_fused_kernel(const u16* __restrict__ X16 ,
                                                             const u16* __restrict__ Wpq_a, const float* __restrict__ bpq,
                                                             const u16* __restrict__ Wpkv_a, const float* __restrict__ bpkv,
                                                             const u16* __restrict__ Wp_a, const float* __restrict__ bp,
                                                             const float* __restrict__ res , float* __restrict__ out,
                                                             RowMap rm, long long Mp, int N_a, int L_a, float scale, const u16* __restrict__ Q16 = nullptr,
                                                             const u16* __restrict__ K16 = nullptr,
                                                             const u16* __restrict__ VT16 = nullptr, FfnArgs fa_a = FfnArgs{},
                                                             const u16* __restrict__ Wk2T_a = nullptr ,
                                                             int wt = 0 ,
                                                             int spatial_only = 0 ,
                                                             const float* __restrict__ ln_g = nullptr ,
                                                             const float* __restrict__ ln_b = nullptr,
                                                             OwnQkv oq_a = OwnQkv{}) {
  static_assert(!FFN || MT == 4, "the FFN half works on 64-row tiles");
  static_assert(MQ == 0 || ((MT == 4 || MT == 2 || MT == 1) && NKS > 0), "own q/k/v: 64-, 32- or 16-row tiles");
  static_assert(MQ != 2 || (MT == 4 && NKS == 2 && T >= 2), "own frame first: a 64-row tile is one 64-key frame");
  constexpr int C = 256, ROWS = MT * 16;
  extern __shared__ __attribute__((aligned(16))) u16 smem[];
  u16* xt = smem;
  float* sbias = reinterpret_cast<float*>(reinterpret_cast<char*>(smem) + temporal_tile_bytes<T, MT, FFN>());
  float* const sqkvb = sbias + 3 * C + (FFN ? fa_a.F + 5 * C : 0);
  FfnLds fl;
  if constexpr (FFN) {
    fl.ytile = xt;
    fl.xtile = reinterpret_cast<float*>(xt + 8 * ROWS * 32);
    fl.htile = reinterpret_cast<u16*>(fl.xtile + ROWS * kEpiLd);
    fl.par = sbias + 3 * C;
  }

  const int tid = threadIdx.x, lane = tid & 63, wave = tid >> 6;
  const int fi = lane & 15, fg = lane >> 4;
  const int N = N_a, L = L_a;
  const u16* const Wpq = Wpq_a;
  const u16* const Wpkv = Wpkv_a;
  const u16* const Wp = Wp_a;
  const u16* const Wk2T = Wk2T_a;
  const FfnArgs& fa = fa_a;
  const OwnQkv& oq = oq_a;
  long long tile = blockIdx.x;
  long long m0;
  int nvalid;
  if constexpr (NKS > 0) {
    const int tps = (N + ROWS - 1) / ROWS;
    if (gridDim.x % (8 * tps) == 0) {
      const int xcd = blockIdx.x & 7, j = blockIdx.x >> 3;
      tile = ((long long)(j / tps) * 8 + xcd) * tps + (j % tps);
    }
    const long long sq = tile / tps;
    const int n0 = (int)(tile - sq * tps) * ROWS;
    m0 = sq * N + n0;
    nvalid = min(ROWS, N - n0);
  } else {
    m0 = tile * ROWS;
    nvalid = (int)min((long long)ROWS, Mp - m0);
  }

  [[maybe_unused]] const int Lr = rm.Lv ? rm.Lv : L;
  AXVS_STAMP_DECL;
  AXVS_WG_BEGIN;
  AXVS_STAMP(0);
  auto stage_small = [&]() {
    if (tid < C) {
      sbias[tid] = bpq[tid];
      sbias[C + tid] = bpkv[C + tid];
      sbias[2 * C + tid] = bp[tid];
    }
    if constexpr (FFN) {
      lds_fence();
      ffn_stage_params(fl, fa.b1, fa.b2, fa.g1, fa.be1, fa.g2, fa.be2, fa.F, tid);
    }
  };
  u16x8 wf[2][8];
  if constexpr (NKS == 0) load_wfrags<2, 8>(wf, Wpq, C, 0, wave * 32, fi, fg);

  if constexpr (NKS > 0) {
    const long long seq0 = (m0 / N) * N;
    const u16* Qh = Q16 + (long long)wave * Mp * 32;
    const u16* Kh = K16 + (long long)wave * Mp * 32;
    const long long nsf = Mp / L;
    const u16* Vh = VT16 + (long long)wave * nsf * NKS * 1024;
    u16x8 qf[MT];
    u16x8 kb[2][2 * NKS], vf[2][NKS];
    [[maybe_unused]] const ScBuf kbuf(K16), vbuf(VT16);
    [[maybe_unused]] unsigned kvo[2 * NKS], vvo = 0;
    [[maybe_unused]] const unsigned kstep_b = (unsigned)L * 64u, vstep_b = NKS * 2048u;
    [[maybe_unused]] unsigned* const cnt = MQ != 0 ? oq.sync + m0 / N : nullptr;
    [[maybe_unused]] const unsigned tps_u = (unsigned)((N + ROWS - 1) / ROWS);
    [[maybe_unused]] u16x8 vown[2][NKS];
    [[maybe_unused]] float poison = 1.f;
    auto wait_siblings = [&]() {
      unsigned spins = 0;
      while (ld_sc1_u32(cnt) < tps_u) {
        __builtin_amdgcn_s_sleep(2);
        if (++spins > oq.spin_limit) {
          if (oq.status != nullptr && lane == 0) atomicOr(oq.status, 4);
          poison = __uint_as_float(__builtin_amdgcn_readfirstlane(0x7fc00000u));
          break;
        }
      }
    };
    if constexpr (MQ != 0) {
      constexpr int KBSq = ROWS * 32;
      u16* const tqk = xt;
      u16* const tv = xt + 8 * KBSq;
      float sm3[3], sq3[3], sf5[5], sf1[2];
      auto request_params = [&]() {
        load_wfrags<2, 8>(wf, oq.Wv, C, 0, wave * 32, fi, fg);
        if (tid < C) {
          sq3[0] = oq.bq[tid]; sq3[1] = oq.bk[tid]; sq3[2] = oq.bv[tid];
          sm3[0] = bpq[tid]; sm3[1] = bpkv[C + tid]; sm3[2] = bp[tid];
          if constexpr (FFN) {
            sf5[0] = fa.b2[tid]; sf5[1] = fa.g1[tid]; sf5[2] = fa.be1[tid]; sf5[3] = fa.g2[tid]; sf5[4] = fa.be2[tid];
          }
        }
        if constexpr (FFN) {
#pragma unroll
          for (int i = 0; i < 2; ++i)
            if (tid + i * 512 < fa.F) sf1[i] = fa.b1[tid + i * 512];
        }
      };
      {
        constexpr int RPWq = ROWS / 8;
        constexpr int GRPq = RPWq >= 4 ? 4 : RPWq;
        int off_lo, off_hi, coords = 0;
        {
          const int myrow = wave + 8 * (lane & (RPWq - 1));
          const int mym = (int)m0 + min(myrow, nvalid - 1);
          const long long myoff = (oq.pg.mode ? nat_row_coords(rm, mym, oq.pg.l_is_h, &coords) : nat_row(rm, mym)) * C;
          off_lo = (int)(myoff & 0xffffffffll);
          off_hi = (int)(myoff >> 32);
        }
        PosGenLane pl;
        if (oq.pg.mode) pl.init(oq.pg, lane * 4);
        float amax = 0.f;
#pragma unroll
        for (int half = 0; half < RPWq / GRPq; ++half) {
          float4 a[GRPq], p[GRPq];
#pragma unroll
          for (int i = 0; i < GRPq; ++i) {
            const int k = half * GRPq + i;
            const long long off = (((long long)__builtin_amdgcn_readlane(off_hi, k) << 32) | (unsigned)__builtin_amdgcn_readlane(off_lo, k)) + lane * 4;
            a[i] = *reinterpret_cast<const float4*>(oq.src + off);
            if (oq.pg.mode) p[i] = pl.eval(oq.pg, __builtin_amdgcn_readlane(coords, k));
            else p[i] = oq.pos ? *reinterpret_cast<const float4*>(oq.pos + off) : float4{0.f, 0.f, 0.f, 0.f};
          }
          if (half == 0) request_params();
#pragma unroll
          for (int i = 0; i < GRPq; ++i) {
            const int row = wave + 8 * (half * GRPq + i);
            const int n = lane * 4, kbq = n >> 5, k = n & 31;
            const int o = (kbq * ROWS + row) * 32 + swz_chunk(row, k >> 3) * 8 + (k & 7);
            *reinterpret_cast<u16x4*>(tv + o) = cvt4<BF>(f32x4{a[i].x, a[i].y, a[i].z, a[i].w});
            *reinterpret_cast<u16x4*>(tqk + o) = cvt4<BF>(f32x4{a[i].x + p[i].x, a[i].y + p[i].y, a[i].z + p[i].z, a[i].w + p[i].w});
            if (!BF) {
              amax = fmaximum(amax, fmaximum(fmaximum(fabsf(a[i].x), fabsf(a[i].y)), fmaximum(fabsf(a[i].z), fabsf(a[i].w))));
              amax = fmaximum(amax, fmaximum(fmaximum(fabsf(a[i].x + p[i].x), fabsf(a[i].y + p[i].y)), fmaximum(fabsf(a[i].z + p[i].z), fabsf(a[i].w + p[i].w))));
            }
          }
          lds_fence();
        }
        if (!BF && oq.status != nullptr && !(amax <= 65504.f)) atomicOr(oq.status, 1);
      }
      if (tid < C) {
        sqkvb[tid] = sq3[0]; sqkvb[C + tid] = sq3[1]; sqkvb[2 * C + tid] = sq3[2];
        sbias[tid] = sm3[0]; sbias[C + tid] = sm3[1]; sbias[2 * C + tid] = sm3[2];
        if constexpr (FFN) {
          float* q = fl.par + fa.F;
          q[tid] = sf5[0]; q[256 + tid] = sf5[1]; q[512 + tid] = sf5[2]; q[768 + tid] = sf5[3]; q[1024 + tid] = sf5[4];
        }
      }
      lds_fence();
      if constexpr (FFN) {
#pragma unroll
        for (int i = 0; i < 2; ++i)
          if (tid + i * 512 < fa.F) fl.par[tid + i * 512] = sf1[i];
        lds_fence();
        for (int i = tid + 1024; i < fa.F; i += 512) {
          fl.par[i] = fa.b1[i];
          lds_fence();
        }
      }
      AXVS_STAMP(16);
      __syncthreads();
      AXVS_STAMP(17);
      int bb[MT];
#pragma unroll
      for (int mt = 0; mt < MT; ++mt) {
        const int row = mt * 16 + fi;
        bb[mt] = row * 32 + swz_chunk(row, fg) * 8;
      }
      const WtBuf wkb(K16), wvb(VT16);
      {
        f32x4 acc[2][MT];
#pragma unroll
        for (int a = 0; a < 2; ++a)
#pragma unroll
          for (int b = 0; b < MT; ++b) acc[a][b] = f32x4{0.f, 0.f, 0.f, 0.f};
        sweep8<BF, MT, true, true>(acc, wf, tv, bb, KBSq, oq.Wk, C, wave * 32, fi, fg);
        if (MT >= 2 && L % 32 == 0) {
#pragma unroll
          for (int nt = 0; nt < 2; ++nt) {
            const float b = sqkvb[2 * C + wave * 32 + nt * 16 + fi];
#pragma unroll
            for (int mp = 0; mp + 1 < MT; mp += 2) {
              float v[8] = {acc[nt][mp][0] + b, acc[nt][mp][1] + b, acc[nt][mp][2] + b, acc[nt][mp][3] + b,
                            acc[nt][mp + 1][0] + b, acc[nt][mp + 1][1] + b, acc[nt][mp + 1][2] + b, acc[nt][mp + 1][3] + b};
              const u16x8 v8 = cvt8<BF>(v);
              if constexpr (MQ == 2) vown[nt][mp >> 1] = v8;
              if (mp * 16 < nvalid) {
                const unsigned mt0 = (unsigned)m0 + mp * 16;
                const unsigned sf = mt0 / (unsigned)L;
                const int ks = (int)(mt0 - sf * L) >> 5;
                const long long d = ((((long long)wave * nsf + sf) * NKS + ks) * 2 + nt) * 512 + fi * 32 + fg * 8;
                wvb.store16((unsigned)(d * 2), v8);
              }
            }
          }
        } else {
#pragma unroll
          for (int nt = 0; nt < 2; ++nt) {
            const float b = sqkvb[2 * C + wave * 32 + nt * 16 + fi];
#pragma unroll
            for (int mt = 0; mt < MT; ++mt) {
              if (mt * 16 < nvalid) {
                const unsigned mt0 = (unsigned)m0 + mt * 16;
                const unsigned sf = mt0 / (unsigned)L;
                const int l = (int)(mt0 - sf * L) + fg * 4;
                const int ks = l >> 5, pp = fg * 8 + ((l >> 4) & 1) * 4;
                const long long d = ((((long long)wave * nsf + sf) * NKS + ks) * 2 + nt) * 512 + fi * 32 + pp;
                f32x4 v = acc[nt][mt];
                v[0] += b; v[1] += b; v[2] += b; v[3] += b;
                wvb.store8((unsigned)(d * 2), cvt4<BF>(v));
                if (L % 32 != 0 && (int)(mt0 - sf * L) + 16 == L) wvb.store8((unsigned)((d ^ 4) * 2), u16x4{0, 0, 0, 0});
              }
            }
          }
        }
      }
      AXVS_STAMP(18);
      {
        f32x4 acc[2][MT];
#pragma unroll
        for (int a = 0; a < 2; ++a)
#pragma unroll
          for (int b = 0; b < MT; ++b) acc[a][b] = f32x4{0.f, 0.f, 0.f, 0.f};
        sweep8<BF, MT, true>(acc, wf, tqk, bb, KBSq, oq.Wq, C, wave * 32, fi, fg);
        const float4 b0 = *reinterpret_cast<const float4*>(sqkvb + C + wave * 32 + fg * 4);
        const float4 b1 = *reinterpret_cast<const float4*>(sqkvb + C + wave * 32 + 16 + fg * 4);
#pragma unroll
        for (int mt = 0; mt < MT; ++mt) {
          float v[8] = {acc[0][mt][0] + b0.x, acc[0][mt][1] + b0.y, acc[0][mt][2] + b0.z, acc[0][mt][3] + b0.w,
                        acc[1][mt][0] + b1.x, acc[1][mt][1] + b1.y, acc[1][mt][2] + b1.z, acc[1][mt][3] + b1.w};
          const u16x8 k8 = cvt8<BF>(v);
          if constexpr (MQ == 2) kb[0][mt] = k8;
          if (mt * 16 + fi < nvalid) wkb.store16((unsigned)((((long long)wave * Mp + m0 + mt * 16 + fi) * 32 + fg * 8) * 2), k8);
        }
      }
      AXVS_STAMP(19);
      vm_drain();
      AXVS_STAMP(20);
      __syncthreads();
      if (tid == 0) atomicInc(cnt, 2 * tps_u - 1);
      AXVS_STAMP(21);
      if (spatial_only == 2) {
        if (tid == 0) atomicInc(cnt, 2 * tps_u - 1);
        return;
      }
      {
        f32x4 acc[2][MT];
#pragma unroll
        for (int a = 0; a < 2; ++a)
#pragma unroll
          for (int b = 0; b < MT; ++b) acc[a][b] = f32x4{0.f, 0.f, 0.f, 0.f};
        sweep8<BF, MT, false>(acc, wf, tqk, bb, KBSq, oq.Wq, C, 0, fi, fg);
        const float4 b0 = *reinterpret_cast<const float4*>(sqkvb + wave * 32 + fg * 4);
        const float4 b1 = *reinterpret_cast<const float4*>(sqkvb + wave * 32 + 16 + fg * 4);
        const float sc_ = oq.qscale;
#pragma unroll
        for (int mt = 0; mt < MT; ++mt) {
          float v[8] = {(acc[0][mt][0] + b0.x) * sc_, (acc[0][mt][1] + b0.y) * sc_, (acc[0][mt][2] + b0.z) * sc_, (acc[0][mt][3] + b0.w) * sc_,
                        (acc[1][mt][0] + b1.x) * sc_, (acc[1][mt][1] + b1.y) * sc_, (acc[1][mt][2] + b1.z) * sc_, (acc[1][mt][3] + b1.w) * sc_};
          qf[mt] = cvt8<BF>(v);
        }
      }
      AXVS_STAMP(22);
      __syncthreads();
#pragma unroll
      for (int kt = 0; kt < 2 * NKS; ++kt)
        kvo[kt] = (unsigned)((((long long)wave * Mp + seq0 + min(kt * 16 + fi, Lr - 1)) * 32 + fg * 8) * 2);
      vvo = (unsigned)((((long long)wave * nsf + seq0 / L) * (NKS * 1024) + fi * 32 + fg * 8) * 2);
      if constexpr (MQ == 1) {
        wait_siblings();
        AXVS_STAMP(23);
#pragma unroll
        for (int kt = 0; kt < 2 * NKS; ++kt) kb[0][kt] = kbuf.load16(kvo[kt], 0);
      }
    } else {
#pragma unroll
    for (int qt = 0; qt < MT; ++qt) qf[qt] = *reinterpret_cast<const u16x8*>(Qh + (m0 + min(qt * 16 + fi, nvalid - 1)) * 32 + fg * 8);
    }
    const bool ragged = Lr != NKS * 32;
    u16x8 ones;
#pragma unroll
    for (int j = 0; j < 8; ++j) ones[j] = H16<BF>::from_f32(1.f);
    const u16* kp[2 * NKS];
#pragma unroll
    for (int kt = 0; kt < 2 * NKS; ++kt) kp[kt] = Kh + (seq0 + min(kt * 16 + fi, Lr - 1)) * 32 + fg * 8;
    const u16* vp = Vh + (seq0 / L) * (NKS * 1024) + fi * 32 + fg * 8;
    const int kstep = L * 32;
    if constexpr (MQ == 0) {
#pragma unroll
    for (int kt = 0; kt < 2 * NKS; ++kt) kb[0][kt] = *reinterpret_cast<const u16x8*>(kp[kt]);
    }
    AXVS_STAMP(11);
    if constexpr (MQ == 0) stage_small();
#ifdef AXVS_STAMPS
    int nvis_ = 0;
#endif
    auto frame = [&](const int f, const int fnext, auto par_tag, auto last_tag, auto own_tag, auto vpre_tag) {
      constexpr int PAR = decltype(par_tag)::value;
      constexpr bool LAST = decltype(last_tag)::value;
      constexpr bool OWN = decltype(own_tag)::value;
      constexpr bool VPRE = decltype(vpre_tag)::value;
      if constexpr (MQ != 0) {
        if constexpr (!OWN) {
          if constexpr (!VPRE) {
#pragma unroll
            for (int nd = 0; nd < 2; ++nd)
#pragma unroll
              for (int ks = 0; ks < NKS; ++ks) vf[nd][ks] = vbuf.load16(vvo + (ks * 2 + nd) * 1024, (unsigned)f * vstep_b);
          }
          if constexpr (!LAST) {
#pragma unroll
            for (int kt = 0; kt < 2 * NKS; ++kt) kb[PAR ^ 1][kt] = kbuf.load16(kvo[kt], (unsigned)fnext * kstep_b);
          }
        }
      } else {
#pragma unroll
      for (int nd = 0; nd < 2; ++nd)
#pragma unroll
        for (int ks = 0; ks < NKS; ++ks) vf[nd][ks] = *reinterpret_cast<const u16x8*>(vp + (ks * 2 + nd) * 512);
      vp += NKS * 1024;
      if constexpr (!LAST) {
#pragma unroll
        for (int kt = 0; kt < 2 * NKS; ++kt) kp[kt] += kstep;
#pragma unroll
        for (int kt = 0; kt < 2 * NKS; ++kt) kb[PAR ^ 1][kt] = *reinterpret_cast<const u16x8*>(kp[kt]);
      }
      }
      f32x4 sc[MT][2 * NKS];
#pragma unroll
      for (int kt = 0; kt < 2 * NKS; ++kt) {
#pragma unroll
        for (int qt = 0; qt < MT; ++qt) sc[qt][kt] = H16<BF>::mfma(kb[PAR][kt], qf[qt], f32x4{0.f, 0.f, 0.f, 0.f});
      }
      if constexpr (OWN) {
        AXVS_STAMP(23);
        wait_siblings();
#pragma unroll
        for (int kt = 0; kt < 2 * NKS; ++kt) kb[PAR ^ 1][kt] = kbuf.load16(kvo[kt], (unsigned)fnext * kstep_b);
#pragma unroll
        for (int nd = 0; nd < 2; ++nd)
#pragma unroll
          for (int ks = 0; ks < NKS; ++ks) vf[nd][ks] = vbuf.load16(vvo + (ks * 2 + nd) * 1024, (unsigned)fnext * vstep_b);
        AXVS_STAMP(11);
      }
      if (ragged) {
#pragma unroll
        for (int kt = 0; kt < 2 * NKS; ++kt)
#pragma unroll
          for (int r = 0; r < 4; ++r)
            if (kt * 16 + fg * 4 + r >= Lr) {
#pragma unroll
              for (int qt = 0; qt < MT; ++qt) sc[qt][kt][r] = -INFINITY;
            }
      }
      float inv[MT];
      u16x8 pf[MT][NKS];
#pragma unroll
      for (int qt = 0; qt < MT; ++qt) {
        float mx = sc[qt][0][0];
#pragma unroll
        for (int kt = 0; kt < 2 * NKS; ++kt)
#pragma unroll
// ... 40 lines not shown
#ifdef AXVS_STAMPS
      {
        const int v_ = MQ == 2 ? nvis_++ : f;
        if (v_ == 0) { AXVS_STAMP(12); } else if (v_ == 1) { AXVS_STAMP(13); } else if (v_ == 2) { AXVS_STAMP(14); } else { AXVS_STAMP(15); }
      }
#endif
    };
    {
      using I0 = std::integral_constant<int, 0>;
      using I1 = std::integral_constant<int, 1>;
      using F_ = std::false_type;
      using T_ = std::true_type;
      if constexpr (MQ == 2) {
        const int fown = (int)(m0 - seq0) / L;
        auto fr = [&](int i) { const int f = fown + i; return f >= T ? f - T : f; };
        frame(fr(0), fr(1), I0{}, F_{}, T_{}, F_{});
        if constexpr (T > 2) {
          frame(fr(1), fr(2), I1{}, F_{}, F_{}, T_{});
          int i = 2;
#pragma nounroll
          for (; i + 2 <= T - 1; i += 2) {
            frame(fr(i), fr(i + 1), I0{}, F_{}, F_{}, F_{});
            frame(fr(i + 1), fr(i + 2), I1{}, F_{}, F_{}, F_{});
          }
          if constexpr (((T - 3) & 1) != 0) frame(fr(T - 2), fr(T - 1), std::integral_constant<int, (T - 2) & 1>{}, F_{}, F_{}, F_{});
          frame(fr(T - 1), 0, std::integral_constant<int, (T - 1) & 1>{}, T_{}, F_{}, F_{});
        } else {
          frame(fr(1), 0, I1{}, T_{}, F_{}, T_{});
        }
      } else {
      int f = 0;
#pragma nounroll
      for (; f + 2 <= T - 1; f += 2) {
        frame(f, f + 1, I0{}, F_{}, F_{}, F_{});
        frame(f + 1, f + 2, I1{}, F_{}, F_{}, F_{});
      }
      if constexpr (((T - 1) & 1) != 0) frame(T - 2, T - 1, I0{}, F_{}, F_{}, F_{});
      frame(T - 1, 0, std::integral_constant<int, (T - 1) & 1>{}, T_{}, F_{}, F_{});
      }
    }
    if constexpr (MQ == 0) {
      if (spatial_only) return;
    }
  } else {
  {
    constexpr int NCH = T * 8 * ROWS * 4;
    constexpr int PER = (NCH + 511) / 512;
    const int mrow_max = nvalid - 1;
    u16x8 v[PER];
#pragma unroll
    for (int p = 0; p < PER; ++p) {
      const int c = min(tid + p * 512, NCH - 1);
      const int g = c & 3, row = (c >> 2) % ROWS, blk = (c >> 2) / ROWS;
      const int f = blk >> 3, kb = blk & 7;
      v[p] = *reinterpret_cast<const u16x8*>(X16 + (((long long)(kb * T + f)) * Mp + m0 + min(row, mrow_max)) * 32 + g * 8);
    }
#pragma unroll
    for (int p = 0; p < PER; ++p) {
      const int c = tid + p * 512;
      if (c < NCH) {
        const int g = c & 3, row = (c >> 2) % ROWS, blk = (c >> 2) / ROWS;
        *reinterpret_cast<u16x8*>(xt + (blk * ROWS + row) * 32 + swz_chunk(row, g) * 8) = v[p];
      }
      if ((p & 7) == 7) lds_fence();
    }
  }
  }
  if constexpr (NKS == 0) stage_small();
  __syncthreads();
  if constexpr (MQ != 0) {
    const int tps = (N + ROWS - 1) / ROWS;
    if (tid == 0) atomicInc(oq.sync + m0 / N, 2 * (unsigned)tps - 1);
    if (spatial_only) return;
  }

  AXVS_STAMP(1);
  int bown[MT], bfr[MT];
  {
    const int mrow = (int)m0 + min(lane, nvalid - 1);
    const int fown_l = (int)(((unsigned)mrow % (unsigned)N) / (unsigned)L);
#pragma unroll
    for (int mt = 0; mt < MT; ++mt) {
      const int row = mt * 16 + fi;
      const int fown = __builtin_amdgcn_ds_bpermute(row * 4, fown_l);
      bown[mt] = xt_off<MT>(fown, 0, row, fg);
      bfr[mt] = xt_off<MT>(0, 0, row, fg);
    }
  }
  constexpr int KBS = ROWS * 32;
  constexpr int FS = 8 * ROWS * 32;

  f32x4 q2[2][MT];
#pragma unroll
  for (int a = 0; a < 2; ++a)
#pragma unroll
    for (int b = 0; b < MT; ++b) q2[a][b] = f32x4{0.f, 0.f, 0.f, 0.f};
  sweep8<BF, MT, true>(q2, wf, xt, bown, KBS, Wk2T, 32, wave * C, fi, fg);
#pragma unroll
  for (int nt = 0; nt < 2; ++nt) {
    const float4 b = *reinterpret_cast<const float4*>(sbias + wave * 32 + nt * 16 + fg * 4);
#pragma unroll
    for (int mt = 0; mt < MT; ++mt) {
      q2[nt][mt][0] = (q2[nt][mt][0] + b.x) * scale; q2[nt][mt][1] = (q2[nt][mt][1] + b.y) * scale;
      q2[nt][mt][2] = (q2[nt][mt][2] + b.z) * scale; q2[nt][mt][3] = (q2[nt][mt][3] + b.w) * scale;
    }
  }

  AXVS_STAMP(2);
  u16x8 q2f[MT];
#pragma unroll
  for (int mt = 0; mt < MT; ++mt) {
    float v[8] = {q2[0][mt][0], q2[0][mt][1], q2[0][mt][2], q2[0][mt][3], q2[1][mt][0], q2[1][mt][1], q2[1][mt][2], q2[1][mt][3]};
    q2f[mt] = cvt8<BF>(v);
  }
  float lg[T][MT];
  f32x4 lacc[T][MT];
#pragma unroll
  for (int f = 0; f < T; ++f)
#pragma unroll
    for (int mt = 0; mt < MT; ++mt) lacc[f][mt] = f32x4{0.f, 0.f, 0.f, 0.f};
  {
    constexpr int PD = T <= 4 ? 2 : 1;
    u16x8 xg[PD + 1][T];
#pragma unroll
    for (int g0 = 0; g0 < PD; ++g0)
#pragma unroll
      for (int f = 0; f < T; ++f) xg[g0][f] = *reinterpret_cast<const u16x8*>(xt + bfr[g0 % MT] + f * FS + (g0 / MT) * KBS);
#pragma unroll
    for (int kb = 0; kb < 8; ++kb) {
      f32x4 qk[2][MT];
#pragma unroll
      for (int nt = 0; nt < 2; ++nt)
#pragma unroll
        for (int mt = 0; mt < MT; ++mt) qk[nt][mt] = H16<BF>::mfma(wf[nt][kb], q2f[mt], f32x4{0.f, 0.f, 0.f, 0.f});
#pragma unroll
      for (int nt = 0; nt < 2; ++nt) wf[nt][kb] = w_frag(Wpkv, 2 * C, kb, C + wave * 32 + nt * 16 + fi, fg);
#pragma unroll
      for (int mt = 0; mt < MT; ++mt) {
        const int g = kb * MT + mt;
        if (g + PD < 8 * MT) {
#pragma unroll
          for (int f = 0; f < T; ++f)
            xg[(g + PD) % (PD + 1)][f] = *reinterpret_cast<const u16x8*>(xt + bfr[(g + PD) % MT] + f * FS + ((g + PD) / MT) * KBS);
        }
        {
          float v8[8] = {qk[0][mt][0], qk[0][mt][1], qk[0][mt][2], qk[0][mt][3], qk[1][mt][0], qk[1][mt][1], qk[1][mt][2], qk[1][mt][3]};
          const u16x8 ua = cvt8<BF>(v8);
          {
#pragma unroll
          for (int f = 0; f < T; ++f) lacc[f][mt] = H16<BF>::mfma(ua, xg[g % (PD + 1)][f], lacc[f][mt]);
          }
        }
        __builtin_amdgcn_sched_barrier(0);
      }
    }
  }
  {
    const int sel = fi & 3, srcl = (fi + 16 * (fi >> 2)) * 4;
#pragma unroll
    for (int f = 0; f < T; ++f)
#pragma unroll
      for (int mt = 0; mt < MT; ++mt) {
        const f32x4 a = lacc[f][mt];
        const float d = sel == 0 ? a[0] : sel == 1 ? a[1] : sel == 2 ? a[2] : a[3];
        lg[f][mt] = __int_as_float(__builtin_amdgcn_ds_bpermute(srcl, __float_as_int(d)));
      }
  }
// ... 4 lines not shown
#pragma unroll
    for (int f = 1; f < T; ++f) mx = fmaxf(mx, lg[f][mt]);
    float s = 0.f;
#pragma unroll
    for (int f = 0; f < T; ++f) {
      lg[f][mt] = __expf(lg[f][mt] - mx);
      s += lg[f][mt];
    }
    const float inv = 1.f / s;
#pragma unroll
    for (int f = 0; f < T; ++f) lg[f][mt] *= inv;
  }

  f32x4 o[2][MT];
#pragma unroll
  for (int nt = 0; nt < 2; ++nt) {
    const float4 b = *reinterpret_cast<const float4*>(sbias + C + wave * 32 + nt * 16 + fg * 4);
#pragma unroll
    for (int mt = 0; mt < MT; ++mt) o[nt][mt] = f32x4{b.x, b.y, b.z, b.w};
  }
  {
    constexpr int PD = T <= 4 ? 2 : 1;
    u16x8 xg[PD + 1][T];
#pragma unroll
    for (int g0 = 0; g0 < PD; ++g0)
#pragma unroll
      for (int f = 0; f < T; ++f) xg[g0][f] = *reinterpret_cast<const u16x8*>(xt + bfr[g0 % MT] + f * FS + (g0 / MT) * KBS);
#pragma unroll
    for (int kb = 0; kb < 8; ++kb) {
      u16x8 xb[MT];
#pragma unroll
      for (int mt = 0; mt < MT; ++mt) {
        const int g = kb * MT + mt;
        if (g + PD < 8 * MT) {
#pragma unroll
          for (int f = 0; f < T; ++f)
            xg[(g + PD) % (PD + 1)][f] = *reinterpret_cast<const u16x8*>(xt + bfr[(g + PD) % MT] + f * FS + ((g + PD) / MT) * KBS);
        }
        u16x8 acc = {0, 0, 0, 0, 0, 0, 0, 0};
#pragma unroll
        for (int f = 0; f < T; ++f) acc = axpy8<BF>(lg[f][mt], xg[g % (PD + 1)][f], acc);
        xb[mt] = acc;
        __builtin_amdgcn_sched_barrier(0);
      }
#pragma unroll
      for (int nt = 0; nt < 2; ++nt)
#pragma unroll
        for (int mt = 0; mt < MT; ++mt) o[nt][mt] = H16<BF>::mfma(wf[nt][kb], xb[mt], o[nt][mt]);
#pragma unroll
      for (int nt = 0; nt < 2; ++nt) wf[nt][kb] = w_frag(Wp, C, kb, wave * 32 + nt * 16 + fi, fg);
      __builtin_amdgcn_sched_barrier(0);
    }
  }

  AXVS_STAMP(4);
  __syncthreads();
  AXVS_STAMP(5);
#pragma unroll
  for (int nt = 0; nt < 2; ++nt)
#pragma unroll
    for (int mt = 0; mt < MT; ++mt) {
      const int n = wave * 32 + nt * 16 + fg * 4, row = mt * 16 + fi;
      *reinterpret_cast<u16x4*>(xt + ((n >> 5) * ROWS + row) * 32 + swz_chunk(row, (n & 31) >> 3) * 8 + (n & 7)) = cvt4<BF>(o[nt][mt]);
    }
  AXVS_STAMP(9);
  __syncthreads();
  AXVS_STAMP(6);
  f32x4 po[2][MT];
#pragma unroll
  for (int a = 0; a < 2; ++a)
#pragma unroll
    for (int b = 0; b < MT; ++b) po[a][b] = f32x4{0.f, 0.f, 0.f, 0.f};
  int bo[MT];
#pragma unroll
  for (int mt = 0; mt < MT; ++mt) {
    const int row = mt * 16 + fi;
    bo[mt] = row * 32 + swz_chunk(row, fg) * 8;
  }
  constexpr int RPW = ROWS / 8;
  float4 rres[RPW];
  long long roff[RPW];
  [[maybe_unused]] int roff_lo = 0, roff_hi = 0;
  unsigned rok;
  {
    const int myrow = wave * RPW + (lane % RPW);
    const int mym = (int)m0 + min(myrow, nvalid - 1);
    rok = (unsigned)__builtin_amdgcn_ballot_w64(myrow < nvalid && row_exists(rm, mym)) & ((1u << RPW) - 1u);
    const long long myoff = nat_row(rm, mym) * C;
    const int lo = (int)(myoff & 0xffffffffll), hi = (int)(myoff >> 32);
    roff_lo = lo;
    roff_hi = hi;
#pragma unroll
    for (int i = 0; i < RPW; ++i) {
      const long long o = ((long long)__builtin_amdgcn_readlane(hi, i) << 32) | (unsigned)__builtin_amdgcn_readlane(lo, i);
      roff[i] = o + lane * 4;
      rres[i] = *reinterpret_cast<const float4*>(res + roff[i]);
    }
  }
  constexpr int crot = 0;
  if constexpr (FFN) sweep8<BF, MT, true>(po, wf, xt, bo, KBS, fa.W1, fa.F, crot * 256 + wave * 32, fi, fg);
  else sweep8<BF, MT, false>(po, wf, xt, bo, KBS, Wp, C, 0, fi, fg);
  AXVS_STAMP(7);
  float* etile = reinterpret_cast<float*>(xt + 8 * ROWS * 32);
#pragma unroll
  for (int nt = 0; nt < 2; ++nt) {
    const int n = wave * 32 + nt * 16 + fg * 4;
    const float4 b = *reinterpret_cast<const float4*>(sbias + 2 * C + n);
#pragma unroll
    for (int mt = 0; mt < MT; ++mt)
      epi_put(etile, mt * 16 + fi, n, f32x4{po[nt][mt][0] + b.x, po[nt][mt][1] + b.y, po[nt][mt][2] + b.z, po[nt][mt][3] + b.w});
  }
  __syncthreads();
  [[maybe_unused]] NoRows yrows;
#pragma unroll
  for (int i = 0; i < RPW; ++i) {
    const int row = wave * RPW + i;
    const float4 v = *reinterpret_cast<const float4*>(etile + row * kEpiLd + lane * 4);
    float4 y = float4{v.x + rres[i].x, v.y + rres[i].y, v.z + rres[i].z, v.w + rres[i].w};
    if constexpr (!FFN) {
      if (ln_g) {
        const float mu = wave_sum(y.x + y.y + y.z + y.w) * (1.f / C);
        const float d0 = y.x - mu, d1 = y.y - mu, d2 = y.z - mu, d3 = y.w - mu;
        const float rstd = rsqrtf(wave_sum(d0 * d0 + d1 * d1 + d2 * d2 + d3 * d3) * (1.f / C) + 1e-5f);
        const float4 g = *reinterpret_cast<const float4*>(ln_g + lane * 4), b = *reinterpret_cast<const float4*>(ln_b + lane * 4);
        y = float4{d0 * rstd * g.x + b.x, d1 * rstd * g.y + b.y, d2 * rstd * g.z + b.z, d3 * rstd * g.w + b.w};
      }
    }
    if constexpr (FFN) yrows.v[i] = y;
    else if ((rok >> i) & 1u) {
      if (wt & 1) WtBuf(out).store16((unsigned)(roff[i] * 4), y);
      else *reinterpret_cast<float4*>(out + roff[i]) = y;
    }
  }
  AXVS_STAMP(8);
  if constexpr (FFN) {
    static_assert(RPW == 8, "the FFN half walks 8 rows per wave");
    auto row_off_ = [=](int row) { return ((rok >> (row % RPW)) & 1u) ? roff[row % RPW] - lane * 4 : -1ll; };
    ffn_body<BF, decltype(row_off_), false, true>(fl, wf, fa.W1, fa.W2, out, row_off_, fa.F, 0, crot, tid, wt, yrows);
  }
  AXVS_STAMP(10);
  AXVS_WG_END(FFN ? 0 : 1);
#if !defined(AXVS_STAMPS_QKV) && !defined(AXVS_STAMPS_FFN)
  if constexpr (MQ != 0 && !FFN) AXVS_STAMP_FLUSH_AT(32, 24);
  else if constexpr (MQ != 0) AXVS_STAMP_FLUSH(24);
  else AXVS_STAMP_FLUSH(16);
#endif
}


}

#if defined(AXVS_STAMPS) && defined(AXVS_STAMPS_QKV)
#define QSTAMP_DECL AXVS_STAMP_DECL
#define QSTAMP(s) AXVS_STAMP(s)
#define QSTAMP_FLUSH(n) AXVS_STAMP_FLUSH(n)
#else
#define QSTAMP_DECL
#define QSTAMP(s)
#define QSTAMP_FLUSH(n)
#endif
namespace axvs {

template <bool BF>
__global__ __launch_bounds__(512) void qkv_fused_kernel(const float* __restrict__ src, const float* __restrict__ pos, RowMap rm,
                                                        const u16* __restrict__ Wq, const u16* __restrict__ Wk,
                                                        const u16* __restrict__ Wv, const float* __restrict__ bq,
                                                        const float* __restrict__ bk, const float* __restrict__ bv,
                                                        u16* __restrict__ Q16, u16* __restrict__ K16, u16* __restrict__ V16,
                                                        long long Mp, float qscale, u16* __restrict__ VT16, int N, int L, int T,
                                                        int NKS, PosGen pg, int wt ,
                                                        int* __restrict__ status ) {
  constexpr int C = 256, MT = 4, ROWS = 64, KBS = ROWS * 32;
  extern __shared__ __attribute__((aligned(16))) u16 smem[];
  u16* tqk = smem;
  u16* tv = smem + 8 * KBS;
  float* sbias = reinterpret_cast<float*>(smem + 16 * KBS);
  const int tid = threadIdx.x, lane = tid & 63, wave = tid >> 6;
  const int fi = lane & 15, fg = lane >> 4;
  const long long m0 = (long long)blockIdx.x * ROWS;

  QSTAMP_DECL;
  QSTAMP(0);
  const WtBuf wq(Q16), wk(K16), wvt(VT16), wvr(V16);
  const bool split = gridDim.y == 3;
  const int part = split ? (int)blockIdx.y : 0;
  u16x8 wf[2][8];
  load_wfrags<2, 8>(wf, part == 0 ? Wq : part == 1 ? Wk : Wv, C, 0, wave * 32, fi, fg);
  float bias3[3];
  if (tid < C) {
    bias3[0] = bq[tid]; bias3[1] = bk[tid]; bias3[2] = bv[tid];
  }

  {
    const int c4 = tid & 63;
    int off_lo, off_hi, coords = 0;
    {
      const int myrow = (tid >> 6) + 8 * (lane & 7);
      const long long mym = min(m0 + myrow, Mp - 1);
      const long long myoff = (pg.mode ? nat_row_coords(rm, (int)mym, pg.l_is_h, &coords) : nat_row(rm, (int)mym)) * C;
      off_lo = (int)(myoff & 0xffffffffll);
      off_hi = (int)(myoff >> 32);
    }
    PosGenLane pl;
    if (pg.mode) pl.init(pg, c4 * 4);
    float amax = 0.f;
#pragma unroll
    for (int half = 0; half < 2; ++half) {
      float4 a[4], p[4];
#pragma unroll
      for (int i = 0; i < 4; ++i) {
        const int k = half * 4 + i;
        const long long off = (((long long)__builtin_amdgcn_readlane(off_hi, k) << 32) | (unsigned)__builtin_amdgcn_readlane(off_lo, k)) + c4 * 4;
        a[i] = *reinterpret_cast<const float4*>(src + off);
        if (pg.mode) p[i] = pl.eval(pg, __builtin_amdgcn_readlane(coords, k));
        else p[i] = pos ? *reinterpret_cast<const float4*>(pos + off) : float4{0.f, 0.f, 0.f, 0.f};
      }
#pragma unroll
      for (int i = 0; i < 4; ++i) {
        const int row = (tid >> 6) + 8 * (half * 4 + i);
        const int n = c4 * 4, kb = n >> 5, k = n & 31;
        const int o = (kb * ROWS + row) * 32 + swz_chunk(row, k >> 3) * 8 + (k & 7);
// ... 151 lines not shown
```

axial_vs_amd/csrc/axvs_host.h:

```cpp
#pragma once
#include <hip/hip_runtime.h>

#include <cstdarg>
#include <cstdio>

#include "../../include/axvs.h"
#include "axvs_common.h"

namespace axvs {

inline thread_local char g_err[512] = "";
inline int g_train_valu = 0;
inline int g_train_exact = 1;
inline int g_train_amp = 0;
inline int g_spatial_wgs = 512;
inline int g_train_attn_split = 1;

inline thread_local int g_cc_aspp_affine = 0;
inline thread_local int g_cc_last_only = 0;

inline thread_local hipEvent_t* g_prof_events = nullptr;
inline thread_local int g_prof_cap = 0;
inline thread_local int g_prof_next = 0;
constexpr int kMaxStages = 32;
inline thread_local const char* g_stage_names[kMaxStages] = {};
inline void mark(hipStream_t st, const char* name) {
  if (g_prof_next < kMaxStages) g_stage_names[g_prof_next] = name;
  if (g_prof_events && g_prof_next < g_prof_cap) (void)hipEventRecord(g_prof_events[g_prof_next], st);
  ++g_prof_next;
}

inline int fail(int code, const char* fmt, ...) {
  va_list ap;
  va_start(ap, fmt);
  vsnprintf(g_err, sizeof(g_err), fmt, ap);
  va_end(ap);
  return code;
}

inline int last_launch_status() {
  hipError_t e = hipGetLastError();
  if (e != hipSuccess) return fail(AXVS_ERR_LAUNCH, "HIP launch failed: %s", hipGetErrorString(e));
  return AXVS_OK;
}

inline size_t align_up(size_t x, size_t a = 256) { return (x + a - 1) / a * a; }

struct Carver {
  char* base;
  size_t off = 0;
  explicit Carver(void* p) : base(static_cast<char*>(p)) {}
  template <class T>
  T* take(size_t n) {
    T* p = base ? reinterpret_cast<T*>(base + off) : nullptr;
    off = align_up(off + n * sizeof(T));
    return p;
  }
  float* f(size_t n) { return take<float>(n); }
};

template <class F>
size_t carved(F&& step) {
  Carver c(nullptr);
  step(c);
  return c.off;
}

inline int check_ws(size_t have, size_t need) {
  if (have < need) return fail(AXVS_ERR_WORKSPACE, "workspace too small: %zu < %zu", have, need);
  return AXVS_OK;
}
inline int check_ws(long long have, size_t need) {
  if (have < 0 || (size_t)have < need) return fail(AXVS_ERR_WORKSPACE, "workspace too small: %lld < %zu", have, need);
  return AXVS_OK;
}

inline int ensure_max_lds(const void* fn) {
  constexpr int kCap = 256;
  struct Entry { int dev; const void* fn; };
  static thread_local Entry seen[kCap];
  static thread_local int nseen = 0;
  int dev = 0;
  if (hipGetDevice(&dev) != hipSuccess) return fail(AXVS_ERR_LAUNCH, "hipGetDevice failed");
  for (int i = 0; i < nseen; ++i)
    if (seen[i].fn == fn && seen[i].dev == dev) return AXVS_OK;
  hipFuncAttributes fa;
  if (hipFuncGetAttributes(&fa, fn) != hipSuccess) return fail(AXVS_ERR_LAUNCH, "hipFuncGetAttributes failed");
  const int bytes = 160 * 1024 - (int)((fa.sharedSizeBytes + 255) / 256 * 256);
  if (hipFuncSetAttribute(fn, hipFuncAttributeMaxDynamicSharedMemorySize, bytes) != hipSuccess)
    return fail(AXVS_ERR_LAUNCH, "hipFuncSetAttribute failed");
  if (nseen < kCap) seen[nseen++] = Entry{dev, fn};
  return AXVS_OK;
}

struct TrajPacked {
  u16 *wq, *wk, *wv, *wpq, *wpkv, *wp, *wk2t;
  u16 *wk2n, *wv2h;
  float *bq, *bk, *bv, *bpq, *bpkv, *bp;
  const float *post_ln_g = nullptr, *post_ln_b = nullptr;
};

struct TrajWs {
  u16 *q16, *k16, *v16, *x16, *o16, *vt16;
  float *q2, *kv2;
};

// ... 10 lines not shown
```

axial_vs_amd/csrc/axvs_infer.h:

```cpp
#pragma once
#include <type_traits>

#include "axvs_host.h"
#include "axvs_gemm.h"

namespace axvs {

#ifdef AXVS_WITH_BF16
constexpr bool kBF = true;
#else
constexpr bool kBF = false;
#endif
inline int check_dtype(int dtype) {
  if (dtype == AXVS_F16) return AXVS_OK;
  if (dtype == AXVS_BF16) {
    if (kBF) return AXVS_OK;
    return fail(AXVS_ERR_ARG, "the bf16 operand tier is not built into this library (it does not hold the 1e-3 parity bar; fp16 operands run at the same rate and do): rebuild with AXVS_WITH_BF16=1");
  }
  return fail(AXVS_ERR_ARG, "unknown dtype %d", dtype);
}
template <class F>
auto by_dtype(int dtype, F&& f) {
  return dtype == AXVS_BF16 ? f(std::bool_constant<kBF>{}) : f(std::false_type{});
}
// ... 37 lines not shown
  t.bp = c.take<float>(C);
  return t;
}

struct LayerPacked {
  TrajPacked th, tw;
  u16 *w1, *w2;
  float *b1, *b2, *g1, *be1, *g2, *be2;
};

inline LayerPacked carve_ffn(Carver& c, int C, int F) {
  LayerPacked l{};
  l.w1 = c.take<u16>((size_t)F * C);
  l.w2 = c.take<u16>((size_t)F * C);
  l.b1 = c.take<float>(F);
  l.b2 = c.take<float>(C);
  l.g1 = c.take<float>(C);
  l.be1 = c.take<float>(C);
  l.g2 = c.take<float>(C);
  l.be2 = c.take<float>(C);
  return l;
}

inline LayerPacked carve_layer(Carver& c, int C, int heads, int F) {
  const TrajPacked th = carve_traj(c, C, heads), tw = carve_traj(c, C, heads);
  LayerPacked l = carve_ffn(c, C, F);
  l.th = th;
  l.tw = tw;
  return l;
}

void pack_w(int dtype, const float* W, u16* out, PackDim nd, PackDim kd, hipStream_t st, int n_off = 0, int n_total = 0);
void pack_w3(int dtype, const float* W, u16* out, PackDim nd, PackDim kd, hipStream_t st, int n_off = 0, int n_total = 0);
void pack_b(const float* b, float* out, PackDim nd, hipStream_t st);
void copy_f32(const float* src, float* dst, int n, hipStream_t st);
void pack_traj(int dtype, const AxvsTrajParams& p, const TrajPacked& t, int C, int heads, hipStream_t st);
void pack_ffn(int dtype, const float* n1w, const float* n1b, const float* l1w, const float* l1b, const float* l2w, const float* l2b,
              const float* n2w, const float* n2b, const LayerPacked& l, int C, int F, hipStream_t st);
template <class P>
void pack_ffn(int dtype, const P& p, const LayerPacked& l, int C, int F, hipStream_t st) {
  pack_ffn(dtype, p.norm1_w, p.norm1_b, p.linear1_w, p.linear1_b, p.linear2_w, p.linear2_b, p.norm2_w, p.norm2_b, l, C, F, st);
}

inline int pad16(int L) { return (L + 15) & ~15; }
inline long long padded_rows(long long M, int L) { return L > 0 && L % 16 ? M / L * pad16(L) : M; }

inline TrajWs carve_traj_ws(Carver& c, long long Mp, int T, int heads, bool lean = false, long long Mq = 0) {
  const size_t Cp = (size_t)heads * 32;
  if (Mq < Mp) Mq = Mp;
  TrajWs w{};
  w.q16 = c.take<u16>(Cp * Mq);
  w.k16 = c.take<u16>(Cp * Mq);
  w.vt16 = c.take<u16>(2 * Cp * Mq);
  if (lean) return w;
  w.v16 = c.take<u16>(Cp * Mp);
  w.x16 = c.take<u16>(Cp * Mp * T);
  w.o16 = c.take<u16>(Cp * Mp);
  w.q2 = c.take<float>(Cp * Mp);
  w.kv2 = c.take<float>(((size_t)2 * Cp * T > (size_t)2 * heads * Cp ? (size_t)2 * Cp * T : (size_t)2 * heads * Cp) * Mp);
  return w;
}

struct FfnWs {
  float *x, *tmp;
  u16 *y16, *h16;
};
inline FfnWs carve_ffn_ws(Carver& c, long long M, int C, int F) {
  FfnWs w{};
  w.x = c.take<float>((size_t)M * C);
  w.tmp = c.take<float>((size_t)M * C);
  w.y16 = c.take<u16>((size_t)M * C);
  w.h16 = c.take<u16>((size_t)M * F);
  return w;
}

struct TrajPlan {
  enum Tier { kFused, kTemporalFused, kGeneric } tier;
  enum Qkv { kQkvKernel, kQkvKernel3, kQkvGemms } qkv;
  int L;
  int nks;
  int rows;
  int mq;
  bool with_ffn;
  bool reassoc;
  bool may_merge;
};
TrajPlan plan_traj(int S, int T, int L, int C, int heads, bool want_attn, bool same_src, int F, bool may_merge);

int run_traj(int dtype, const TrajPlan& pl, const float* qsrc, const float* ksrc, const float* vsrc, const float* qk_add, const float* res,
             float* out, float* attn, const TrajPacked& p, const TrajWs& w, RowMap rm, int S, int T, int L, int C, int heads, hipStream_t st);

int ffn_rows(int dtype, const FfnWs& w, float* out, const LayerPacked& p, long long M, int C, int heads, int d_ffn, hipStream_t st);
int ffn_rows(int dtype, const float* x, float* out, const LayerPacked& p, long long M, int C, int heads, int d_ffn, void* workspace, hipStream_t st);

void layernorm_rows(int dtype, const float* X, const float* gamma, const float* beta, float* Y, u16* Y16, long long M, int C, hipStream_t st);

extern template void launch_gemm<false, ALoadBlocked<false>, EpiBlocked16<false>>(const ALoadBlocked<false>&, const u16*, const EpiBlocked16<false>&, int, int, int, hipStream_t, int);
#ifdef AXVS_WITH_BF16
extern template void launch_gemm<true, ALoadBlocked<true>, EpiBlocked16<true>>(const ALoadBlocked<true>&, const u16*, const EpiBlocked16<true>&, int, int, int, hipStream_t, int);
#endif

}
```

axial_vs_amd/csrc/axvs_temporal_inst.hip:

```cpp
#include "axvs_host.h"
#include "axvs_fused.h"

#if !defined(AXVS_INST_BF) || !defined(AXVS_INST_T)
#error "compile with -DAXVS_INST_BF=<0|1> -DAXVS_INST_T=<frames> [-DAXVS_INST_MT=<16-row tiles per workgroup>]"
#endif
#ifndef AXVS_INST_MT
#define AXVS_INST_MT (AXVS_INST_T <= 4 ? 4 : 2)
#endif

namespace axvs {

template <bool BF, int T, int MT, int NKS, bool FFN, int MQ = 0>
static int launch_one(unsigned grid, const TrajWs& w, const TrajPacked& p, const float* res, float* out, RowMap rm, long long Mp, int N, int L,
                      float scale, hipStream_t st, const FfnArgs* fa, int wt, const OwnQkv* oq = nullptr) {
  auto kern = &temporal_fused_kernel<BF, T, MT, NKS, FFN, MQ>;
  if (int rc = ensure_max_lds(reinterpret_cast<const void*>(kern))) return rc;
  const size_t lds = temporal_lds_bytes<T, MT, FFN, MQ>(FFN ? fa->F : 0);
  hipLaunchKernelGGL(kern, dim3(grid), dim3(512), lds, st, w.x16, p.wpq, p.bpq, p.wpkv, p.bpkv, p.wp, p.bp, res, out, rm, Mp, N, L, scale,
                     w.q16, w.k16, w.vt16, FFN ? *fa : FfnArgs{}, p.wk2t, (wt & 1) | (FFN ? wt & kOut16Mask : 0), (wt >> 1) & 3, FFN ? nullptr : p.post_ln_g,
                     FFN ? nullptr : p.post_ln_b, MQ ? *oq : OwnQkv{});
  return AXVS_OK;
}

template <bool BF, int T, int MT, int NKS>
static int launch_temporal_t(const TrajWs& w, const TrajPacked& p, const float* res, float* out, RowMap rm, long long Mp, int N, int L,
                             float scale, hipStream_t st, const FfnArgs* fa, int wt, const OwnQkv* oq) {
  const unsigned grid = NKS > 0 ? (unsigned)((Mp / N) * ((N + MT * 16 - 1) / (MT * 16))) : (unsigned)((Mp + MT * 16 - 1) / (MT * 16));
  if constexpr (NKS > 0 && NKS <= 3 && MT == 4 && T <= 4) {
    if (oq) {
      if constexpr (NKS == 2 && T >= 2) {
        if (L == 64) {
          if (fa) return launch_one<BF, T, MT, NKS, true, 2>(grid, w, p, res, out, rm, Mp, N, L, scale, st, fa, wt, oq);
          return launch_one<BF, T, MT, NKS, false, 2>(grid, w, p, res, out, rm, Mp, N, L, scale, st, fa, wt, oq);
        }
      }
      if (fa) return launch_one<BF, T, MT, NKS, true, 1>(grid, w, p, res, out, rm, Mp, N, L, scale, st, fa, wt, oq);
      return launch_one<BF, T, MT, NKS, false, 1>(grid, w, p, res, out, rm, Mp, N, L, scale, st, fa, wt, oq);
    }
  }
  if constexpr (NKS > 0 && MT == 1 && T <= 4) {
    if (oq) {
      if (fa) return fail(AXVS_ERR_ARG, "internal: merged q/k/v on 16-row tiles excludes the FFN");
      return launch_one<BF, T, MT, NKS, false, 1>(grid, w, p, res, out, rm, Mp, N, L, scale, st, fa, wt, oq);
    }
  }
  if constexpr (NKS > 0 && NKS <= 3 && MT == 2 && T >= 5) {
    if (oq) {
      if (fa) return fail(AXVS_ERR_ARG, "internal: merged q/k/v on 32-row tiles excludes the FFN");
      return launch_one<BF, T, MT, NKS, false, 1>(grid, w, p, res, out, rm, Mp, N, L, scale, st, fa, wt, oq);
    }
  }
  if (oq) return fail(AXVS_ERR_ARG, "internal: merged q/k/v needs the in-kernel spatial half on 64- / 16-row tiles (T <= 4) or 32-row tiles (T = 5 .. 8)");
  if constexpr (NKS > 0 && MT == 4) {
    if (fa) return launch_one<BF, T, MT, NKS, true>(grid, w, p, res, out, rm, Mp, N, L, scale, st, fa, wt);
  }
  if (fa) return fail(AXVS_ERR_ARG, "internal: FFN fusion needs the in-kernel spatial half and 64-row tiles");
  return launch_one<BF, T, MT, NKS, false>(grid, w, p, res, out, rm, Mp, N, L, scale, st, fa, wt);
}

template <bool BF, int T, int MT>
int launch_temporal_n(int nks, const TrajWs& w, const TrajPacked& p, const float* res, float* out, RowMap rm, long long Mp, int N,
                      int L, float scale, hipStream_t st, const FfnArgs* fa, int wt, const OwnQkv* oq) {
  switch (nks) {
    case 0: return launch_temporal_t<BF, T, MT, 0>(w, p, res, out, rm, Mp, N, L, scale, st, fa, wt, oq);
    case 1: return launch_temporal_t<BF, T, MT, 1>(w, p, res, out, rm, Mp, N, L, scale, st, fa, wt, oq);
    case 2: return launch_temporal_t<BF, T, MT, 2>(w, p, res, out, rm, Mp, N, L, scale, st, fa, wt, oq);
    case 3: return launch_temporal_t<BF, T, MT, 3>(w, p, res, out, rm, Mp, N, L, scale, st, fa, wt, oq);
    case 4: return launch_temporal_t<BF, T, MT, 4>(w, p, res, out, rm, Mp, N, L, scale, st, fa, wt, oq);
    default: return fail(AXVS_ERR_ARG, "bad nks");
  }
}

template int launch_temporal_n<(AXVS_INST_BF != 0), AXVS_INST_T, AXVS_INST_MT>(
    int, const TrajWs&, const TrajPacked&, const float*, float*, RowMap, long long, int, int, float, hipStream_t, const FfnArgs*, int,
    const OwnQkv*);

}

#if defined(AXVS_STAMPS) && !defined(AXVS_STAMPS_QKV) && AXVS_INST_BF == 0 && AXVS_INST_T == 4 && AXVS_INST_MT == 4
extern "C" int axvs_debug_read_stamps(unsigned long long* host, int n) {
  return (int)hipMemcpyFromSymbol(host, HIP_SYMBOL(axvs::g_stamps), sizeof(unsigned long long) * n);
}
#endif

#if defined(AXVS_STAMPS) && !defined(AXVS_STAMPS_QKV) && AXVS_INST_BF == 0 && AXVS_INST_T == 4 && AXVS_INST_MT == 1
extern "C" int axvs_debug_read_stamps_mt1(unsigned long long* host, int n) {
  return (int)hipMemcpyFromSymbol(host, HIP_SYMBOL(axvs::g_stamps), sizeof(unsigned long long) * n);
}
#endif

#if defined(AXVS_STAMPS_WG) && AXVS_INST_BF == 0 && AXVS_INST_T == 4 && AXVS_INST_MT == 4
extern "C" int axvs_debug_read_wg_times(unsigned long long* host, int n) {
  return (int)hipMemcpyFromSymbol(host, HIP_SYMBOL(axvs::g_wg), sizeof(unsigned long long) * n);
}
#endif
```

include/axvs.h:

```cpp
#ifndef AXVS_H
#define AXVS_H

#include <stddef.h>
#include <stdint.h>

#ifdef __cplusplus
extern "C" {
#endif

#define AXVS_F16 0
#define AXVS_BF16 1
#define AXVS_F32 2
#define AXVS_U8 3

#define AXVS_OK 0
#define AXVS_ERR_ARG (-1)
#define AXVS_ERR_WORKSPACE (-2)
#define AXVS_ERR_LAUNCH (-3)
#define AXVS_ERR_STATE (-4)

typedef struct AxvsTrajParams {
  const float *q_w, *q_b;
  const float *k_w, *k_b;
  const float *v_w, *v_b;
  const float *proj_q_w, *proj_q_b;
  const float *proj_kv_w, *proj_kv_b;
  const float *proj_w, *proj_b;
} AxvsTrajParams;

typedef struct AxvsAxialLayerParams {
  AxvsTrajParams height_attn, width_attn;
  const float *norm1_w, *norm1_b;
  const float *linear1_w, *linear1_b;
  const float *linear2_w, *linear2_b;
  const float *norm2_w, *norm2_b;
} AxvsAxialLayerParams;

int axvs_version(void);
int axvs_has_bf16(void);
const char* axvs_last_error(void);

#define AXVS_STATUS_FP16_RANGE 1
#define AXVS_STATUS_SYNC_TIMEOUT 4
int axvs_set_status_buffer(int* device_word);
int axvs_check_status(void);

int axvs_set_sync_buffer(unsigned* device_words, size_t n_words);

int axvs_profile_stages(void** events, int capacity);
int axvs_profile_stage_count(void);
const char* axvs_profile_stage_name(int i);

int axvs_set_option(const char* key, int value);

size_t axvs_traj_packed_bytes(int C, int heads);
int axvs_traj_pack(const AxvsTrajParams* p, void* packed, int C, int heads, int dtype, void* stream);
size_t axvs_axial_layer_packed_bytes(int C, int heads, int d_ffn);
int axvs_axial_layer_pack(const AxvsAxialLayerParams* p, void* packed, int C, int heads, int d_ffn, int dtype,
                          void* stream);

size_t axvs_traj_attn_workspace_bytes(int S, int T, int L, int C, int heads);
int axvs_traj_attn_fwd(const float* query, const float* key, const float* value, float* out, float* space_attn,
                       const void* packed, int S, int T, int L, int C, int heads, int dtype, void* workspace,
                       size_t workspace_bytes, void* stream);

size_t axvs_axial_layer_workspace_bytes(int B, int T, int H, int W, int C, int heads, int d_ffn);
int axvs_axial_layer_fwd(const float* src, const float* pos, float* out, const void* packed, int B, int T, int H,
                         int W, int C, int heads, int d_ffn, int dtype, void* workspace, size_t workspace_bytes,
                         float* h_attn, float* w_attn, void* stream);

typedef struct AxvsTrajLayerParams {
  AxvsTrajParams temporal_attn;
  const float *norm1_w, *norm1_b, *linear1_w, *linear1_b, *linear2_w, *linear2_b, *norm2_w, *norm2_b;
} AxvsTrajLayerParams;
size_t axvs_traj_layer_packed_bytes(int C, int heads, int d_ffn);
int axvs_traj_layer_pack(const AxvsTrajLayerParams* p, void* packed, int C, int heads, int d_ffn, int dtype, void* stream);
size_t axvs_traj_layer_workspace_bytes(int B, int T, int HW, int C, int heads, int d_ffn);
int axvs_traj_layer_fwd(const float* src, const float* pos, float* out, const void* packed, int B, int T, int HW, int C, int heads,
                        int d_ffn, int dtype, void* workspace, size_t workspace_bytes, void* stream);

int axvs_axial_pass_fwd(const float* src, const float* pos, float* out, const void* packed, int pass, int B, int T, int H, int W,
                        int C, int heads, int d_ffn, int dtype, void* workspace, size_t workspace_bytes, void* stream);

typedef struct AxvsSinePos3D {
  float temperature;
  int normalize;
  float scale;
  const float* level_embed;
} AxvsSinePos3D;
size_t axvs_axial_layer_workspace_bytes_ex(int B, int T, int H, int W, int C, int heads, int d_ffn, int want_attn_maps,
                                           int sine_pos);
size_t axvs_axial_layer_sine3d_workspace_bytes(int B, int T, int H, int W, int C, int heads, int d_ffn);
int axvs_axial_layer_fwd_sine3d(const float* src, const AxvsSinePos3D* pos, float* out, const void* packed, int B, int T, int H,
                                int W, int C, int heads, int d_ffn, int dtype, void* workspace, size_t workspace_bytes,
                                float* h_attn, float* w_attn, void* stream);

int axvs_axial_layer_strided_ok(int C, int heads, int d_ffn);
size_t axvs_axial_layer_workspace_bytes_strided(int B, int T, int H, int W, int C, int heads, int d_ffn, long long frame_stride_rows);
int axvs_axial_layer_fwd_sine3d_strided(const float* src, const AxvsSinePos3D* pos, float* out, const void* packed, int B, int T, int H,
                                        int W, int C, int heads, int d_ffn, int dtype, long long frame_stride_rows, void* workspace,
                                        size_t workspace_bytes, void* stream);

size_t axvs_ffn_workspace_bytes(long long M, int C, int d_ffn);
int axvs_ffn_fwd(const float* x, float* out, const void* packed_layer, long long M, int C, int heads, int d_ffn,
                 int dtype, void* workspace, size_t workspace_bytes, void* stream);

typedef struct AxvsFfnParams {
  const float *norm1_w, *norm1_b;
  const float *linear1_w, *linear1_b;
  const float *linear2_w, *linear2_b;
  const float *norm2_w, *norm2_b;
} AxvsFfnParams;
size_t axvs_ffn_packed_bytes(int C, int d_ffn);
int axvs_ffn_pack(const AxvsFfnParams* p, void* packed, int C, int d_ffn, int dtype, void* stream);
int axvs_ffn_packed_fwd(const float* x, float* out, const void* packed_ffn, long long M, int C, int d_ffn, int dtype, void* workspace,
                        size_t workspace_bytes, void* stream);

typedef struct AxvsFpnLevelParams {
  const float* lateral_w;
  const float *lateral_gn_w, *lateral_gn_b;
  const float* output_w;
  const float *output_gn_w, *output_gn_b;
  const float *mask_w, *mask_b;
} AxvsFpnLevelParams;
size_t axvs_fpn_level_packed_bytes(int Cin, int C, int Cm);
int axvs_fpn_level_pack(const AxvsFpnLevelParams* p, void* packed, int Cin, int C, int Cm, int dtype, void* stream);
size_t axvs_fpn_level_workspace_bytes(int N, int H, int W, int Cin, int C, int groups);
int axvs_fpn_level_fwd(const float* x, const float* up, long long up_batch_stride, long long up_ld, int Hu, int Wu, float* y,
                       float* mask_feature, const void* packed, int N, int H, int W, int Cin, int C, int Cm, int groups, float eps, int dtype,
                       void* workspace, size_t workspace_bytes, void* stream);

typedef struct AxvsBN { const float *w, *b, *mean, *var; } AxvsBN;

typedef struct AxvsCCLayerParams {
  AxvsTrajParams attn;
  const float *norm_w, *norm_b;
// ... 485 lines not shown
```

Measured before the change: 39990.

## Add regular-tile specialization for whole-frame fused temporal kernel

Adds a REG template variant of the fused temporal kernel, used when each 64-row tile is exactly one 64-key frame. In that case row offsets, position coordinates and the frame index are computed arithmetically instead of through readlane/bpermute lookups, and ragged and row-validity checks are dropped. It also hoists the per-frame sinusoidal z term out of the per-row positional evaluation and batches LayerNorm reductions across rows so the cross-lane shuffles interleave. Output form is made a compile-time template parameter for the FFN and epilogue stores. The cost is more kernel instantiations and a larger binary, plus a new query hook that reports which passes took the regular path.

```diff
diff --git a/axial_vs_amd/_lib.py b/axial_vs_amd/_lib.py
--- a/axial_vs_amd/_lib.py
+++ b/axial_vs_amd/_lib.py
@@ -242,6 +242,7 @@
     "axvs_profile_stage_count": (C.c_int, []),
     "axvs_profile_stage_name": (C.c_char_p, [C.c_int]),
     "axvs_set_option": (C.c_int, [C.c_char_p, C.c_int]),
+    "axvs_plan_regular_tiles": (C.c_int, []),
     "axvs_traj_packed_bytes": (C.c_size_t, [C.c_int, C.c_int]),
     "axvs_traj_pack": (C.c_int, [C.POINTER(AxvsTrajParams), _fp, C.c_int, C.c_int, C.c_int, _fp]),
     "axvs_axial_layer_packed_bytes": (C.c_size_t, [C.c_int, C.c_int, C.c_int]),
diff --git a/axial_vs_amd/csrc/axvs_api.hip b/axial_vs_amd/csrc/axvs_api.hip
--- a/axial_vs_amd/csrc/axvs_api.hip
+++ b/axial_vs_amd/csrc/axvs_api.hip
@@ -27,6 +27,7 @@
 thread_local int g_ffn_split_pairs = 1;
 thread_local int g_spatial_only = 0;
 thread_local int g_no_ffn_fusion = 0;
+thread_local int g_no_reg_tiles = 0;
 thread_local int g_no_reassoc = 0;
 thread_local int g_ffn_gelu = 0;
 thread_local unsigned* g_sync = nullptr;
@@ -164,6 +165,7 @@
   const bool merge = p.tier == TrajPlan::kFused && may_merge && !g_no_merge_qkv && g_sync != nullptr && (size_t)S <= g_sync_words &&
                      (T <= 4 || p.rows == 32) && p.nks <= (p.rows == 16 ? 4 : 3) && 2 * (long long)heads * 32 * Mp * 2 < (1ll << 32) && fits();
   p.mq = !merge ? 0 : own_frame ? 2 : 1;
+  p.reg = p.mq == 2 && p.L == L && !g_no_reg_tiles && (g_row_span ? g_row_span : Mp) * 256 * 4 < (1ll << 32) && !(p.with_ffn && g_out_dtype);
   return p;
 }
 namespace {
@@ -265,7 +267,7 @@
 int launch_temporal(const TrajPlan& pl, int nks, const TrajWs& w, const TrajPacked& p, const float* res, float* out, RowMap rm, long long Mp, int N,
                     int T, float scale, hipStream_t st, const FfnArgs* fa = nullptr, const OwnQkv* oq = nullptr) {
   const int wt = ((g_row_span ? g_row_span : Mp) * 256 * 4 < (1ll << 32) ? 1 : 0) | (g_spatial_only && nks > 0 ? (oq ? g_spatial_only : 1) << 1 : 0) |
-                 (fa != nullptr && g_out_dtype ? (g_out_dtype == 1 ? kOutF16 : kOutBf16) : 0);
+                 (fa != nullptr && g_out_dtype ? (g_out_dtype == 1 ? kOutF16 : kOutBf16) : 0) | (pl.reg && oq ? kTrajReg : 0);
   if (oq && !(nks > 0 && T <= 8)) return fail(AXVS_ERR_ARG, "internal: own q,k,v need the in-kernel spatial half and T <= 8");
   return by_int<12>(T, [&](auto t) {
     constexpr int kT = decltype(t)::value;
@@ -302,6 +304,7 @@
   const FfnArgs* const fa = pl.with_ffn ? ffn : nullptr;
   float* const dst = pl.with_ffn ? ffn_out : out;
   const PosGen pg = posgen ? *posgen : PosGen{};
+  g_reg_passes = pass == 2 ? (g_reg_passes & 1) | (pl.mq && pl.reg ? 2 : 0) : (pl.mq && pl.reg ? 1 : 0);
   if (pl.mq) {
     const OwnQkv oq{qsrc, qk_add, pg, p.wq, p.wk, p.wv, p.bq, p.bk, p.bv, qscale, g_sync, g_status, g_sync_spin_limit};
     if (int rc = launch_temporal<BF>(pl, pl.nks, w, p, res, dst, rm, Mp, N, T, scale, st, fa, &oq)) return rc;
@@ -430,10 +433,14 @@
     }
     case FfnPlan::kFused: {
       const int rc = by_gelu(pl.gelu, [&](auto g) {
-        const auto kern = &ffn_fused_kernel<BF, decltype(g)::value>;
-        if (int rc = ensure_max_lds(reinterpret_cast<const void*>(kern))) return rc;
-        hipLaunchKernelGGL(kern, dim3(tiles), dim3(512), ffn_lds_bytes(F), st, X, p.w1, p.b1, p.w2, p.b2, p.g1, p.be1, p.g2, p.be2, out, M, F, rs, pl.oflags);
-        return (int)AXVS_OK;
+        const auto launch = [&](auto of) {
+          const auto kern = &ffn_fused_kernel<BF, decltype(g)::value, decltype(of)::value>;
+          if (int rc = ensure_max_lds(reinterpret_cast<const void*>(kern))) return rc;
+          hipLaunchKernelGGL(kern, dim3(tiles), dim3(512), ffn_lds_bytes(F), st, X, p.w1, p.b1, p.w2, p.b2, p.g1, p.be1, p.g2, p.be2, out, M, F, rs);
+          return (int)AXVS_OK;
+        };
+        return pl.oflags == kOutF16 ? launch(std::integral_constant<int, kOutF16>{})
+               : pl.oflags == kOutBf16 ? launch(std::integral_constant<int, kOutBf16>{}) : launch(std::integral_constant<int, 0>{});
       });
       if (rc != AXVS_OK) return rc;
       break;
@@ -625,6 +632,7 @@
   g_prof_cap = events ? capacity : 0;
   return kMaxStages;
 }
+int axvs_plan_regular_tiles(void) { return g_reg_passes; }
 int axvs_profile_stage_count(void) { return g_prof_next < kMaxStages ? g_prof_next : kMaxStages; }
 const char* axvs_profile_stage_name(int i) { return (i >= 0 && i < kMaxStages && g_stage_names[i]) ? g_stage_names[i] : ""; }
 
@@ -664,6 +672,7 @@
     g_ffn_split_pairs = (value & 8) ? 0 : 1;
     g_merge_small = (value & 16) ? 0 : (value & 32) ? 1 : kMergeSmall;
     g_no_reassoc = (value & 64) ? 1 : 0;
+    g_no_reg_tiles = (value & 128) ? 1 : 0;
     return AXVS_OK;
   }
   return fail(AXVS_ERR_ARG, "unknown option");
diff --git a/axial_vs_amd/csrc/axvs_common.h b/axial_vs_amd/csrc/axvs_common.h
--- a/axial_vs_amd/csrc/axvs_common.h
+++ b/axial_vs_amd/csrc/axvs_common.h
@@ -183,14 +183,19 @@
       lv[0] = lv[1] = lv[2] = lv[3] = 0.f;
     }
   }
-  __device__ __forceinline__ float4 eval(const PosGen& pg, int packed) const {
-    const float z = (float)((packed & 255) + 1) * pg.zs;
+  struct ZTerm { float s0, c0, s1, c1; };
+  __device__ __forceinline__ ZTerm zterm(const PosGen& pg, int t) const {
+    const float z = (float)(t + 1) * pg.zs;
+    const float b0 = __builtin_amdgcn_fractf(z * g0), b1 = __builtin_amdgcn_fractf(z * g1);
+    return ZTerm{__builtin_amdgcn_sinf(b0), __builtin_amdgcn_cosf(b0), __builtin_amdgcn_sinf(b1), __builtin_amdgcn_cosf(b1)};
+  }
+  __device__ __forceinline__ float4 eval_yx(const PosGen& pg, int packed, const ZTerm& zt) const {
     const float u = xside ? (float)(((packed >> 20) & 4095) + 1) * pg.xs : (float)(((packed >> 8) & 4095) + 1) * pg.ys;
     const float a0 = __builtin_amdgcn_fractf(u * f0), a1 = __builtin_amdgcn_fractf(u * f1);
-    const float b0 = __builtin_amdgcn_fractf(z * g0), b1 = __builtin_amdgcn_fractf(z * g1);
-    return float4{__builtin_amdgcn_sinf(a0) + __builtin_amdgcn_sinf(b0) + lv[0], __builtin_amdgcn_cosf(a0) + __builtin_amdgcn_cosf(b0) + lv[1],
-                  __builtin_amdgcn_sinf(a1) + __builtin_amdgcn_sinf(b1) + lv[2], __builtin_amdgcn_cosf(a1) + __builtin_amdgcn_cosf(b1) + lv[3]};
-  }
+    return float4{__builtin_amdgcn_sinf(a0) + zt.s0 + lv[0], __builtin_amdgcn_cosf(a0) + zt.c0 + lv[1],
+                  __builtin_amdgcn_sinf(a1) + zt.s1 + lv[2], __builtin_amdgcn_cosf(a1) + zt.c1 + lv[3]};
+  }
+  __device__ __forceinline__ float4 eval(const PosGen& pg, int packed) const { return eval_yx(pg, packed, zterm(pg, packed & 255)); }
 };
 
 __device__ __forceinline__ long long blk_off(long long R, long long r, int k) {
diff --git a/axial_vs_amd/csrc/axvs_fused.h b/axial_vs_amd/csrc/axvs_fused.h
--- a/axial_vs_amd/csrc/axvs_fused.h
+++ b/axial_vs_amd/csrc/axvs_fused.h
@@ -115,6 +115,80 @@
 #endif
 
 constexpr int kOutF16 = 16, kOutBf16 = 32, kOut16Mask = kOutF16 | kOutBf16;
+constexpr int kTrajReg = 8;
+
+constexpr int kFormBits = 1 | kOut16Mask;
+constexpr int kFormRt = -1;
+template <int OF>
+__device__ __forceinline__ void store_row(float* __restrict__ out, long long off , float4 y) {
+  static_assert(OF >= 0 && (OF & ~kFormBits) == 0, "a compile-time output form");
+  if constexpr ((OF & kOut16Mask) != 0) {
+    const u16x4 h = cvt4<(OF & kOutBf16) != 0>(f32x4{y.x, y.y, y.z, y.w});
+    u16* o16 = reinterpret_cast<u16*>(out);
+    if constexpr ((OF & 1) != 0) WtBuf(o16).store8((unsigned)(off * 2), h);
+    else *reinterpret_cast<u16x4*>(o16 + off) = h;
+  } else if constexpr ((OF & 1) != 0) {
+    WtBuf(out).store16((unsigned)(off * 4), y);
+  } else {
+    *reinterpret_cast<float4*>(out + off) = y;
+  }
+}
+template <int OF, class F>
+__device__ __forceinline__ void by_out_form(int wt, F&& f) {
+  if constexpr (OF >= 0) {
+    f(std::integral_constant<int, OF>{});
+  } else {
+    switch (wt & kFormBits) {
+      case 0: f(std::integral_constant<int, 0>{}); break;
+      case 1: f(std::integral_constant<int, 1>{}); break;
+      case kOutF16: f(std::integral_constant<int, kOutF16>{}); break;
+      case kOutF16 | 1: f(std::integral_constant<int, kOutF16 | 1>{}); break;
+      default:
+        if (wt & 1) f(std::integral_constant<int, kOutBf16 | 1>{});
+        else f(std::integral_constant<int, kOutBf16>{});
+    }
+  }
+}
+template <int R>
+__device__ __forceinline__ void wave_sum_rows(float (&s)[R]) {
+#pragma unroll
+  for (int i = 0; i < R; ++i) s[i] += lane_xor1(s[i]);
+#pragma unroll
+  for (int i = 0; i < R; ++i) s[i] += lane_xor2(s[i]);
+#pragma unroll
+  for (int i = 0; i < R; ++i) s[i] += lane_hmirror(s[i]);
+#pragma unroll
+  for (int i = 0; i < R; ++i) s[i] += lane_mirror(s[i]);
+#pragma unroll
+  for (int i = 0; i < R; ++i) {
+    const auto r = __builtin_amdgcn_permlane16_swap(__float_as_uint(s[i]), __float_as_uint(s[i]), false, false);
+    s[i] = __uint_as_float(r[0]) + __uint_as_float(r[1]);
+  }
+#pragma unroll
+  for (int i = 0; i < R; ++i) {
+    const auto r = __builtin_amdgcn_permlane32_swap(__float_as_uint(s[i]), __float_as_uint(s[i]), false, false);
+    s[i] = __uint_as_float(r[0]) + __uint_as_float(r[1]);
+  }
+}
+template <int R>
+__device__ __forceinline__ void ln_stats_rows(float4 (&v)[R], float (&rstd)[R]) {
+  float s[R];
+#pragma unroll
+  for (int i = 0; i < R; ++i) s[i] = v[i].x + v[i].y + v[i].z + v[i].w;
+  wave_sum_rows<R>(s);
+#pragma unroll
+  for (int i = 0; i < R; ++i) {
+    const float mu = s[i] * (1.f / 256);
+    v[i] = float4{v[i].x - mu, v[i].y - mu, v[i].z - mu, v[i].w - mu};
+    s[i] = v[i].x * v[i].x + v[i].y * v[i].y + v[i].z * v[i].z + v[i].w * v[i].w;
+  }
+  wave_sum_rows<R>(s);
+#pragma unroll
+  for (int i = 0; i < R; ++i) rstd[i] = rsqrtf(s[i] * (1.f / 256) + 1e-5f);
+}
+__device__ __forceinline__ float4 ln_apply(float4 d, float rstd, float4 g, float4 b) {
+  return float4{d.x * rstd * g.x + b.x, d.y * rstd * g.y + b.y, d.z * rstd * g.z + b.z, d.w * rstd * g.w + b.w};
+}
 
 struct FfnLds {
   float* xtile;
@@ -147,7 +221,7 @@
 }
 
 struct NoRows { float4 v[8]; };
-template <bool BF, class RowOff, bool GELU = false, bool PRE = false>
+template <bool BF, class RowOff, bool GELU = false, bool PRE = false, int OF = kFormRt, bool ALL = false>
 __device__ __forceinline__ void ffn_body(const FfnLds& l, u16x8 (&w1f)[2][8], const u16* __restrict__ W1, const u16* __restrict__ W2,
                                          float* __restrict__ out, RowOff row_off, int F, int rot, int crot, int tid, int wt = 0,
                                          const NoRows& pre = NoRows{}) {
@@ -163,18 +237,20 @@
 
   {
     const float4 gg = *reinterpret_cast<const float4*>(sg1 + lane * 4), bb = *reinterpret_cast<const float4*>(sbe1 + lane * 4);
+    float4 v[8];
+    float rstd[8];
+#pragma unroll
+    for (int rr = 0; rr < 8; ++rr) {
+      if constexpr (PRE) v[rr] = pre.v[rr];
+      else v[rr] = *reinterpret_cast<const float4*>(l.xtile + (wave * 8 + rr) * kEpiLd + lane * 4);
+    }
+    ln_stats_rows<8>(v, rstd);
 #pragma unroll
     for (int rr = 0; rr < 8; ++rr) {
       const int r = wave * 8 + rr;
-      float4 v;
-      if constexpr (PRE) v = pre.v[rr];
-      else v = *reinterpret_cast<const float4*>(l.xtile + r * kEpiLd + lane * 4);
-      const float mu = wave_sum(v.x + v.y + v.z + v.w) * (1.f / C);
-      const float a = v.x - mu, b = v.y - mu, c = v.z - mu, d = v.w - mu;
-      const float rstd = rsqrtf(wave_sum(a * a + b * b + c * c + d * d) * (1.f / C) + 1e-5f);
-      const f32x4 y = {a * rstd * gg.x + bb.x, b * rstd * gg.y + bb.y, c * rstd * gg.z + bb.z, d * rstd * gg.w + bb.w};
-      *reinterpret_cast<float4*>(l.xtile + r * kEpiLd + lane * 4) = float4{y[0], y[1], y[2], y[3]};
-      act_store4<BF>(l.ytile, lane * 4, r, y);
+      const float4 y = ln_apply(v[rr], rstd[rr], gg, bb);
+      *reinterpret_cast<float4*>(l.xtile + r * kEpiLd + lane * 4) = y;
+      act_store4<BF>(l.ytile, lane * 4, r, f32x4{y.x, y.y, y.z, y.w});
       if (rr == 3) lds_fence();
     }
   }
@@ -283,27 +359,18 @@
   FSTAMP(11);
   {
     const float4 g2v = *reinterpret_cast<const float4*>(sg2 + lane * 4), be2v = *reinterpret_cast<const float4*>(sbe2 + lane * 4);
-#pragma unroll
-    for (int i = 0; i < 8; ++i) {
-      const int r = wave * 8 + i;
-      const float4 v = *reinterpret_cast<const float4*>(l.xtile + r * kEpiLd + lane * 4);
-      const float mu = wave_sum(v.x + v.y + v.z + v.w) * (1.f / C);
-      const float d0 = v.x - mu, d1 = v.y - mu, d2 = v.z - mu, d3 = v.w - mu;
-      const float rstd = rsqrtf(wave_sum(d0 * d0 + d1 * d1 + d2 * d2 + d3 * d3) * (1.f / C) + 1e-5f);
-      const long long off = row_off(r);
-      if (off >= 0) {
-        const float4 y = float4{d0 * rstd * g2v.x + be2v.x, d1 * rstd * g2v.y + be2v.y, d2 * rstd * g2v.z + be2v.z, d3 * rstd * g2v.w + be2v.w};
-        if (wt & kOut16Mask) {
-          const f32x4 yv = {y.x, y.y, y.z, y.w};
-          const u16x4 h = (wt & kOutBf16) ? cvt4<true>(yv) : cvt4<false>(yv);
-          u16* o16 = reinterpret_cast<u16*>(out);
-          if (wt & 1) WtBuf(o16).store8((unsigned)((off + lane * 4) * 2), h);
-          else *reinterpret_cast<u16x4*>(o16 + off + lane * 4) = h;
-        } else if (wt & 1) WtBuf(out).store16((unsigned)((off + lane * 4) * 4), y);
-        else *reinterpret_cast<float4*>(out + off + lane * 4) = y;
-      }
-      if (i == 3) lds_fence();
-    }
+    float4 v[8];
+    float rstd[8];
+#pragma unroll
+    for (int i = 0; i < 8; ++i) v[i] = *reinterpret_cast<const float4*>(l.xtile + (wave * 8 + i) * kEpiLd + lane * 4);
+    ln_stats_rows<8>(v, rstd);
+    by_out_form<OF>(wt, [&](auto form) {
+#pragma unroll
+      for (int i = 0; i < 8; ++i) {
+        const long long off = row_off(wave * 8 + i);
+        if (ALL || off >= 0) store_row<decltype(form)::value>(out, off + lane * 4, ln_apply(v[i], rstd[i], g2v, be2v));
+      }
+    });
   }
   FSTAMP(12);
   FSTAMP_FLUSH(16);
@@ -323,13 +390,13 @@
 #endif
 }
 
-template <bool BF, bool GELU = false>
+template <bool BF, bool GELU = false, int OF = 0>
 __global__ __launch_bounds__(512) void ffn_fused_kernel(const float* __restrict__ X, const u16* __restrict__ W1,
                                                         const float* __restrict__ b1, const u16* __restrict__ W2,
                                                         const float* __restrict__ b2, const float* __restrict__ g1,
                                                         const float* __restrict__ be1, const float* __restrict__ g2,
                                                         const float* __restrict__ be2, float* __restrict__ out,
-                                                        long long M, int F, RowStride rs, int oflags = 0 ) {
+                                                        long long M, int F, RowStride rs) {
   constexpr int C = 256, KB = 8;
   extern __shared__ __attribute__((aligned(16))) char smem_c[];
   FfnLds l;
@@ -359,7 +426,7 @@
   }
   __syncthreads();
   auto row_off = [=](int r) { return m0 + r < M ? rs.row(m0 + r) * C : -1ll; };
-  ffn_body<BF, decltype(row_off), GELU>(l, w1f, W1, W2, out, row_off, F, rot, crot, tid, oflags);
+  ffn_body<BF, decltype(row_off), GELU, false, OF>(l, w1f, W1, W2, out, row_off, F, rot, crot, tid);
 }
 
 constexpr size_t kFfnTiles = (size_t)kRows * kEpiLd * sizeof(float) + 2 * 8 * kTileElems * sizeof(u16);
@@ -431,7 +498,7 @@
   }
 }
 
-template <bool BF, int T, int MT, int NKS = 0, bool FFN = false, int MQ = 0>
+template <bool BF, int T, int MT, int NKS = 0, bool FFN = false, int MQ = 0, bool REG = false>
 __global__ __launch_bounds__(512) void temporal_fused_kernel(const u16* __restrict__ X16 ,
                                                              const u16* __restrict__ Wpq_a, const float* __restrict__ bpq,
                                                              const u16* __restrict__ Wpkv_a, const float* __restrict__ bpkv,
@@ -449,6 +516,7 @@
   static_assert(!FFN || MT == 4, "the FFN half works on 64-row tiles");
   static_assert(MQ == 0 || ((MT == 4 || MT == 2 || MT == 1) && NKS > 0), "own q/k/v: 64-, 32- or 16-row tiles");
   static_assert(MQ != 2 || (MT == 4 && NKS == 2 && T >= 2), "own frame first: a 64-row tile is one 64-key frame");
+  static_assert(!REG || MQ == 2, "regular tiles: a 64-row tile is one whole frame");
   constexpr int C = 256, ROWS = MT * 16;
   extern __shared__ __attribute__((aligned(16))) u16 smem[];
   u16* xt = smem;
@@ -464,7 +532,7 @@
 
   const int tid = threadIdx.x, lane = tid & 63, wave = tid >> 6;
   const int fi = lane & 15, fg = lane >> 4;
-  const int N = N_a, L = L_a;
+  const int N = REG ? T * 64 : N_a, L = REG ? 64 : L_a;
   const u16* const Wpq = Wpq_a;
   const u16* const Wpkv = Wpkv_a;
   const u16* const Wp = Wp_a;
@@ -474,6 +542,8 @@
   long long tile = blockIdx.x;
   long long m0;
   int nvalid;
+  [[maybe_unused]] int rg_f = 0, rg_o = 0;
+  [[maybe_unused]] long long rg_row0 = 0;
   if constexpr (NKS > 0) {
     const int tps = (N + ROWS - 1) / ROWS;
     if (gridDim.x % (8 * tps) == 0) {
@@ -483,13 +553,19 @@
     const long long sq = tile / tps;
     const int n0 = (int)(tile - sq * tps) * ROWS;
     m0 = sq * N + n0;
-    nvalid = min(ROWS, N - n0);
+    nvalid = REG ? ROWS : min(ROWS, N - n0);
+    if constexpr (REG) {
+      const int s = (int)sq, b = s / rm.Loff;
+      rg_f = n0 / ROWS;
+      rg_o = s - b * rm.Loff;
+      rg_row0 = b * rm.sB + rg_f * rm.sT + rg_o * rm.sO;
+    }
   } else {
     m0 = tile * ROWS;
     nvalid = (int)min((long long)ROWS, Mp - m0);
   }
 
-  [[maybe_unused]] const int Lr = rm.Lv ? rm.Lv : L;
+  [[maybe_unused]] const int Lr = REG ? L : rm.Lv ? rm.Lv : L;
   AXVS_STAMP_DECL;
   AXVS_WG_BEGIN;
   AXVS_STAMP(0);
@@ -556,16 +632,31 @@
       {
         constexpr int RPWq = ROWS / 8;
         constexpr int GRPq = RPWq >= 4 ? 4 : RPWq;
-        int off_lo, off_hi, coords = 0;
-        {
+        [[maybe_unused]] int off_lo = 0, off_hi = 0, coords = 0;
+        if constexpr (!REG) {
           const int myrow = wave + 8 * (lane & (RPWq - 1));
           const int mym = (int)m0 + min(myrow, nvalid - 1);
           const long long myoff = (oq.pg.mode ? nat_row_coords(rm, mym, oq.pg.l_is_h, &coords) : nat_row(rm, mym)) * C;
           off_lo = (int)(myoff & 0xffffffffll);
           off_hi = (int)(myoff >> 32);
         }
+        [[maybe_unused]] const int wave_u = __builtin_amdgcn_readfirstlane(wave);
+        auto row_src = [&](int k, long long& off, int& co) {
+          if constexpr (REG) {
+            const int l = wave_u + 8 * k;
+            off = (rg_row0 + l * rm.sL) * C + lane * 4;
+            co = rg_f | ((oq.pg.l_is_h ? l : rg_o) << 8) | ((oq.pg.l_is_h ? rg_o : l) << 20);
+          } else {
+            off = (((long long)__builtin_amdgcn_readlane(off_hi, k) << 32) | (unsigned)__builtin_amdgcn_readlane(off_lo, k)) + lane * 4;
+            co = __builtin_amdgcn_readlane(coords, k);
+          }
+        };
         PosGenLane pl;
-        if (oq.pg.mode) pl.init(oq.pg, lane * 4);
+        [[maybe_unused]] PosGenLane::ZTerm zt{};
+        if (oq.pg.mode) {
+          pl.init(oq.pg, lane * 4);
+          if constexpr (REG) zt = pl.zterm(oq.pg, rg_f);
+        }
         float amax = 0.f;
 #pragma unroll
         for (int half = 0; half < RPWq / GRPq; ++half) {
@@ -573,9 +664,11 @@
 #pragma unroll
           for (int i = 0; i < GRPq; ++i) {
             const int k = half * GRPq + i;
-            const long long off = (((long long)__builtin_amdgcn_readlane(off_hi, k) << 32) | (unsigned)__builtin_amdgcn_readlane(off_lo, k)) + lane * 4;
+            long long off;
+            int co;
+            row_src(k, off, co);
             a[i] = *reinterpret_cast<const float4*>(oq.src + off);
-            if (oq.pg.mode) p[i] = pl.eval(oq.pg, __builtin_amdgcn_readlane(coords, k));
+            if (oq.pg.mode) p[i] = REG ? pl.eval_yx(oq.pg, co, zt) : pl.eval(oq.pg, co);
             else p[i] = oq.pos ? *reinterpret_cast<const float4*>(oq.pos + off) : float4{0.f, 0.f, 0.f, 0.f};
           }
           if (half == 0) request_params();
@@ -733,7 +826,7 @@
 #pragma unroll
     for (int qt = 0; qt < MT; ++qt) qf[qt] = *reinterpret_cast<const u16x8*>(Qh + (m0 + min(qt * 16 + fi, nvalid - 1)) * 32 + fg * 8);
     }
-    const bool ragged = Lr != NKS * 32;
+    const bool ragged = !REG && Lr != NKS * 32;
     u16x8 ones;
 #pragma unroll
     for (int j = 0; j < 8; ++j) ones[j] = H16<BF>::from_f32(1.f);
@@ -940,7 +1033,7 @@
 #pragma unroll
     for (int mt = 0; mt < MT; ++mt) {
       const int row = mt * 16 + fi;
-      const int fown = __builtin_amdgcn_ds_bpermute(row * 4, fown_l);
+      const int fown = REG ? rg_f : __builtin_amdgcn_ds_bpermute(row * 4, fown_l);
       bown[mt] = xt_off<MT>(fown, 0, row, fg);
       bfr[mt] = xt_off<MT>(0, 0, row, fg);
     }
@@ -1111,7 +1204,15 @@
   long long roff[RPW];
   [[maybe_unused]] int roff_lo = 0, roff_hi = 0;
   unsigned rok;
-  {
+  if constexpr (REG) {
+    rok = (1u << RPW) - 1u;
+    const int wave_u = __builtin_amdgcn_readfirstlane(wave);
+#pragma unroll
+    for (int i = 0; i < RPW; ++i) {
+      roff[i] = (rg_row0 + (wave_u * RPW + i) * rm.sL) * C + lane * 4;
+      rres[i] = *reinterpret_cast<const float4*>(res + roff[i]);
+    }
+  } else {
     const int myrow = wave * RPW + (lane % RPW);
     const int mym = (int)m0 + min(myrow, nvalid - 1);
     rok = (unsigned)__builtin_amdgcn_ballot_w64(myrow < nvalid && row_exists(rm, mym)) & ((1u << RPW) - 1u);
@@ -1141,31 +1242,39 @@
   }
   __syncthreads();
   [[maybe_unused]] NoRows yrows;
-#pragma unroll
-  for (int i = 0; i < RPW; ++i) {
-    const int row = wave * RPW + i;
-    const float4 v = *reinterpret_cast<const float4*>(etile + row * kEpiLd + lane * 4);
-    float4 y = float4{v.x + rres[i].x, v.y + rres[i].y, v.z + rres[i].z, v.w + rres[i].w};
-    if constexpr (!FFN) {
+  constexpr int TOF = REG ? 1 : kFormRt;
+  {
+    float4 y[RPW];
+#pragma unroll
+    for (int i = 0; i < RPW; ++i) {
+      const float4 v = *reinterpret_cast<const float4*>(etile + (wave * RPW + i) * kEpiLd + lane * 4);
+      y[i] = float4{v.x + rres[i].x, v.y + rres[i].y, v.z + rres[i].z, v.w + rres[i].w};
+    }
+    if constexpr (FFN) {
+#pragma unroll
+      for (int i = 0; i < RPW; ++i) yrows.v[i] = y[i];
+    } else {
       if (ln_g) {
-        const float mu = wave_sum(y.x + y.y + y.z + y.w) * (1.f / C);
-        const float d0 = y.x - mu, d1 = y.y - mu, d2 = y.z - mu, d3 = y.w - mu;
-        const float rstd = rsqrtf(wave_sum(d0 * d0 + d1 * d1 + d2 * d2 + d3 * d3) * (1.f / C) + 1e-5f);
         const float4 g = *reinterpret_cast<const float4*>(ln_g + lane * 4), b = *reinterpret_cast<const float4*>(ln_b + lane * 4);
-        y = float4{d0 * rstd * g.x + b.x, d1 * rstd * g.y + b.y, d2 * rstd * g.z + b.z, d3 * rstd * g.w + b.w};
-      }
-    }
-    if constexpr (FFN) yrows.v[i] = y;
-    else if ((rok >> i) & 1u) {
-      if (wt & 1) WtBuf(out).store16((unsigned)(roff[i] * 4), y);
-      else *reinterpret_cast<float4*>(out + roff[i]) = y;
+        float rstd[RPW];
+        ln_stats_rows<RPW>(y, rstd);
+#pragma unroll
+        for (int i = 0; i < RPW; ++i) y[i] = ln_apply(y[i], rstd[i], g, b);
+      }
+      const auto store_rows = [&](auto form) {
+#pragma unroll
+        for (int i = 0; i < RPW; ++i)
+          if (REG || ((rok >> i) & 1u)) store_row<decltype(form)::value>(out, roff[i], y[i]);
+      };
+      if (REG || (wt & 1)) store_rows(std::integral_constant<int, 1>{});
+      else store_rows(std::integral_constant<int, 0>{});
     }
   }
   AXVS_STAMP(8);
   if constexpr (FFN) {
     static_assert(RPW == 8, "the FFN half walks 8 rows per wave");
     auto row_off_ = [=](int row) { return ((rok >> (row % RPW)) & 1u) ? roff[row % RPW] - lane * 4 : -1ll; };
-    ffn_body<BF, decltype(row_off_), false, true>(fl, wf, fa.W1, fa.W2, out, row_off_, fa.F, 0, crot, tid, wt, yrows);
+    ffn_body<BF, decltype(row_off_), false, true, TOF, REG>(fl, wf, fa.W1, fa.W2, out, row_off_, fa.F, 0, crot, tid, wt, yrows);
   }
   AXVS_STAMP(10);
   AXVS_WG_END(FFN ? 0 : 1);
diff --git a/axial_vs_amd/csrc/axvs_host.h b/axial_vs_amd/csrc/axvs_host.h
--- a/axial_vs_amd/csrc/axvs_host.h
+++ b/axial_vs_amd/csrc/axvs_host.h
@@ -22,6 +22,7 @@
 inline thread_local hipEvent_t* g_prof_events = nullptr;
 inline thread_local int g_prof_cap = 0;
 inline thread_local int g_prof_next = 0;
+inline thread_local int g_reg_passes = 0;
 constexpr int kMaxStages = 32;
 inline thread_local const char* g_stage_names[kMaxStages] = {};
 inline void mark(hipStream_t st, const char* name) {
diff --git a/axial_vs_amd/csrc/axvs_infer.h b/axial_vs_amd/csrc/axvs_infer.h
--- a/axial_vs_amd/csrc/axvs_infer.h
+++ b/axial_vs_amd/csrc/axvs_infer.h
@@ -143,6 +143,7 @@
   int rows;
   int mq;
   bool with_ffn;
+  bool reg;
   bool reassoc;
   bool may_merge;
 };
diff --git a/axial_vs_amd/csrc/axvs_temporal_inst.hip b/axial_vs_amd/csrc/axvs_temporal_inst.hip
--- a/axial_vs_amd/csrc/axvs_temporal_inst.hip
+++ b/axial_vs_amd/csrc/axvs_temporal_inst.hip
@@ -10,10 +10,10 @@
 
 namespace axvs {
 
-template <bool BF, int T, int MT, int NKS, bool FFN, int MQ = 0>
+template <bool BF, int T, int MT, int NKS, bool FFN, int MQ = 0, bool REG = false>
 static int launch_one(unsigned grid, const TrajWs& w, const TrajPacked& p, const float* res, float* out, RowMap rm, long long Mp, int N, int L,
                       float scale, hipStream_t st, const FfnArgs* fa, int wt, const OwnQkv* oq = nullptr) {
-  auto kern = &temporal_fused_kernel<BF, T, MT, NKS, FFN, MQ>;
+  auto kern = &temporal_fused_kernel<BF, T, MT, NKS, FFN, MQ, REG>;
   if (int rc = ensure_max_lds(reinterpret_cast<const void*>(kern))) return rc;
   const size_t lds = temporal_lds_bytes<T, MT, FFN, MQ>(FFN ? fa->F : 0);
   hipLaunchKernelGGL(kern, dim3(grid), dim3(512), lds, st, w.x16, p.wpq, p.bpq, p.wpkv, p.bpkv, p.wp, p.bp, res, out, rm, Mp, N, L, scale,
@@ -30,6 +30,10 @@
     if (oq) {
       if constexpr (NKS == 2 && T >= 2) {
         if (L == 64) {
+          if (wt & kTrajReg) {
+            if (fa) return launch_one<BF, T, MT, NKS, true, 2, true>(grid, w, p, res, out, rm, Mp, N, L, scale, st, fa, wt, oq);
+            return launch_one<BF, T, MT, NKS, false, 2, true>(grid, w, p, res, out, rm, Mp, N, L, scale, st, fa, wt, oq);
+          }
           if (fa) return launch_one<BF, T, MT, NKS, true, 2>(grid, w, p, res, out, rm, Mp, N, L, scale, st, fa, wt, oq);
           return launch_one<BF, T, MT, NKS, false, 2>(grid, w, p, res, out, rm, Mp, N, L, scale, st, fa, wt, oq);
         }
diff --git a/include/axvs.h b/include/axvs.h
--- a/include/axvs.h
+++ b/include/axvs.h
@@ -52,6 +52,8 @@
 const char* axvs_profile_stage_name(int i);
 
 int axvs_set_option(const char* key, int value);
+
+int axvs_plan_regular_tiles(void);
 
 size_t axvs_traj_packed_bytes(int C, int heads);
 int axvs_traj_pack(const AxvsTrajParams* p, void* packed, int C, int heads, int dtype, void* stream);
```

Result: faster. 41420, median of 6 (+3.6%).
